# uclanlp/visualbert

Measured on NVIDIA H100. Metric: image-text pairs/sec fwd+bwd VisualBERT-base, higher is better.
Workload: dtype bf16

## Files before the change

visualbert_b200/csrc/vb_common.cuh:

```cuda
#pragma once

#include <cuda.h>
#include <cuda_bf16.h>
#include <cuda_runtime.h>
#include <stdint.h>
#include <stdio.h>

#include <atomic>

namespace vb {

typedef __nv_bfloat16 bf16;

extern std::atomic<long long> g_launches;
int num_sms();
constexpr int kMaxDevices = 64;
int current_device();
struct DetWs { void* ptr; long long bytes; };
DetWs det_ws();
int det_require(long long need, const char* what);
const unsigned long long* drop_offset();
template <typename K>
inline cudaError_t ensure_dyn_smem(K kern, int bytes, int (&cache)[kMaxDevices]) {
    const int d = current_device();
    if (cache[d] >= bytes) return cudaSuccess;
    cudaError_t e = cudaFuncSetAttribute(kern, cudaFuncAttributeMaxDynamicSharedMemorySize, bytes);
    if (e == cudaSuccess) cache[d] = bytes;
    return e;
}

enum { PROF_GEMM_FWD = 0, PROF_GEMM_DGRAD = 1, PROF_GEMM_WGRAD = 2, PROF_ATTN_FWD = 3, PROF_ATTN_DQ = 4, PROF_ATTN_DKV = 5,
       PROF_LN_FWD = 6, PROF_LN_BWD = 7, PROF_COLSUM = 8, PROF_EMBED = 9, PROF_OTHER = 10, PROF_NCAT = 11 };
#ifdef __CUDACC__
__device__ __forceinline__ void pdl_wait() { asm volatile("griddepcontrol.wait;" ::: "memory"); }
__device__ __forceinline__ void pdl_trigger() { asm volatile("griddepcontrol.launch_dependents;" ::: "memory"); }
template <typename... KArgs, typename... Args>
inline cudaError_t launch_pdl(void (*kernel)(KArgs...), dim3 grid, dim3 block, size_t smem, cudaStream_t st, Args&&... args) {
    cudaLaunchConfig_t cfg = {};
    cfg.gridDim = grid;
    cfg.blockDim = block;
    cfg.dynamicSmemBytes = smem;
    cfg.stream = st;
    cudaLaunchAttribute attr[1];
    attr[0].id = cudaLaunchAttributeProgrammaticStreamSerialization;
    attr[0].val.programmaticStreamSerializationAllowed = 1;
    cfg.attrs = attr;
    cfg.numAttrs = 1;
    return cudaLaunchKernelEx(&cfg, kernel, static_cast<KArgs>(args)...);
}
#endif

struct ProfScope {
    ProfScope(cudaStream_t st, int cat, double work, int launches);
    ~ProfScope();
    int slot;
    cudaStream_t st;
};

void set_error(const char* fmt, ...);
#define VB_CHECK_CUDA(expr)                                                                   \
    do {                                                                                      \
        cudaError_t _e = (expr);                                                              \
        if (_e != cudaSuccess) {                                                              \
            vb::set_error("%s:%d: %s -> %s", __FILE__, __LINE__, #expr, cudaGetErrorString(_e)); \
            return 1;                                                                         \
        }                                                                                     \
    } while (0)
#define VB_REQUIRE(cond, ...)                                                                 \
    do {                                                                                      \
        if (!(cond)) {                                                                        \
            vb::set_error(__VA_ARGS__);                                                       \
            return 2;                                                                         \
        }                                                                                     \
    } while (0)

#define VB_TRY_RC(expr)      \
    do {                     \
        int _rc = (expr);    \
        if (_rc) return _rc; \
    } while (0)

template <typename... T>
inline bool all_aligned16(const T*... p) {
    return ((reinterpret_cast<uintptr_t>(p) | ... | uintptr_t{0}) & 15) == 0;
}

__device__ __forceinline__ uint32_t smem_u32(const void* p) {
    return static_cast<uint32_t>(__cvta_generic_to_shared(p));
}

__device__ __forceinline__ float warp_sum(float v) {
#pragma unroll
    for (int o = 16; o > 0; o >>= 1) v += __shfl_xor_sync(0xffffffffu, v, o);
    return v;
}
__device__ __forceinline__ float warp_max(float v) {
#pragma unroll
    for (int o = 16; o > 0; o >>= 1) v = fmaxf(v, __shfl_xor_sync(0xffffffffu, v, o));
    return v;
}

__device__ __forceinline__ uint32_t pack_bf16x2(float lo, float hi) {
    __nv_bfloat162 h = __floats2bfloat162_rn(lo, hi);
    return *reinterpret_cast<uint32_t*>(&h);
}
__device__ __forceinline__ float2 unpack_bf16x2(uint32_t v) {
    __nv_bfloat162 h = *reinterpret_cast<__nv_bfloat162*>(&v);
    return __bfloat1622float2(h);
}

__device__ __forceinline__ float fast_ex2(float x) {
    float r;
    asm("ex2.approx.ftz.f32 %0, %1;" : "=f"(r) : "f"(x));
    return r;
}
__device__ __forceinline__ float fast_rcp(float x) {
    float r;
    asm("rcp.approx.ftz.f32 %0, %1;" : "=f"(r) : "f"(x));
    return r;
}

__device__ __forceinline__ float erfc_abs_sqrt2(float x, float& e) {
    const float ax = fabsf(x);
    e = fast_ex2(x * x * -0.72134752044448170f);
    const float t = fast_rcp(fmaf(0.23164189f, ax, 1.0f));
    float poly = fmaf(1.061405429f, t, -1.453152027f);
    poly = fmaf(poly, t, 1.421413741f);
    poly = fmaf(poly, t, -0.284496736f);
    poly = fmaf(poly, t, 0.254829592f);
    return poly * t * e;
}
__device__ __forceinline__ float gelu_fwd(float x) {
    float e;
    const float q = erfc_abs_sqrt2(x, e);
    const float hx = 0.5f * x, ha = fabsf(hx);
    return fmaf(-ha, q, hx + ha);
}
__device__ __forceinline__ void gelu_fwd_bwd(float x, float& g, float& gp) {
    float e;
    const float q = erfc_abs_sqrt2(x, e);
    const float cdf = 0.5f + copysignf(fmaf(-0.5f, q, 0.5f), x);
    g = x * cdf;
    gp = fmaf(x * e, 0.3989422804014327f, cdf);
}
__device__ __forceinline__ float gelu_bwd(float x) {
    float e;
    const float q = erfc_abs_sqrt2(x, e);
    const float cdf = 0.5f + copysignf(fmaf(-0.5f, q, 0.5f), x);
    return fmaf(x * e, 0.3989422804014327f, cdf);
}

__device__ __forceinline__ uint32_t mix32(uint32_t x) {
    x ^= x >> 16; x *= 0x7feb352du;
    x ^= x >> 15; x *= 0x846ca68bu;
    x ^= x >> 16;
    return x;
}
__device__ __forceinline__ uint32_t dropout_key(uint64_t seed, uint32_t stream) {
    return mix32(static_cast<uint32_t>(seed) ^ mix32(static_cast<uint32_t>(seed >> 32) + 0x9E3779B9u * (stream + 1u)));
}
struct DropQ { unsigned thr8; float scale; };
inline DropQ dropout_quantise(float p) {
    DropQ q;
    unsigned n = static_cast<unsigned>(p * 256.0f + 0.5f);
    if (n > 255u) n = 255u;
    q.thr8 = n;
    q.scale = p > 0.f ? 256.0f / (256.0f - static_cast<float>(n)) : 0.f;
    return q;
}
__device__ __forceinline__ uint32_t dropout_keep8_key(uint32_t key0, uint64_t elem8, uint32_t thr8) {
    const uint32_t key = key0 ^ (static_cast<uint32_t>(elem8 >> 31) * 0x27d4eb2fu);
    const uint32_t base = static_cast<uint32_t>(elem8) << 1;
    const uint32_t t4 = thr8 * 0x01010101u;
    const uint32_t m0 = __vcmpgeu4(mix32(base ^ key), t4) & 0x01010101u;
    const uint32_t m1 = __vcmpgeu4(mix32((base + 1u) ^ key), t4) & 0x01010101u;
    return ((m0 * 0x01020408u) >> 24) | (((m1 * 0x01020408u) >> 24) << 4);
}
__device__ __forceinline__ uint32_t dropout_keep8(uint64_t seed, uint32_t stream, uint64_t elem8, uint32_t thr8) {
    return dropout_keep8_key(dropout_key(seed, stream), elem8, thr8);
}

__device__ __forceinline__ void mbar_init(uint32_t bar, uint32_t count) {
    asm volatile("mbarrier.init.shared::cta.b64 [%0], %1;" ::"r"(bar), "r"(count) : "memory");
}
__device__ __forceinline__ void fence_barrier_init() {
    asm volatile("fence.mbarrier_init.release.cluster;" ::: "memory");
}
__device__ __forceinline__ void fence_proxy_async_smem() {
    asm volatile("fence.proxy.async.shared::cta;" ::: "memory");
}
__device__ __forceinline__ void mbar_arrive(uint32_t bar) {
    asm volatile("mbarrier.arrive.shared::cta.b64 _, [%0];" ::"r"(bar) : "memory");
}
__device__ __forceinline__ void mbar_arrive_expect_tx(uint32_t bar, uint32_t bytes) {
    asm volatile("mbarrier.arrive.expect_tx.shared::cta.b64 _, [%0], %1;" ::"r"(bar), "r"(bytes)
                 : "memory");
}
__device__ __forceinline__ bool mbar_try_wait(uint32_t bar, uint32_t parity) {
    uint32_t ok;
    asm volatile(
        "{\n"
        ".reg .pred p;\n"
        "mbarrier.try_wait.parity.shared::cta.b64 p, [%1], %2;\n"
        "selp.u32 %0, 1, 0, p;\n"
        "}\n"
        : "=r"(ok)
        : "r"(bar), "r"(parity)
        : "memory");
    return ok != 0;
}
__device__ __forceinline__ void mbar_wait(uint32_t bar, uint32_t parity) {
    if (mbar_try_wait(bar, parity)) return;
    const long long t0 = clock64();
    uint32_t spins = 0;
    while (!mbar_try_wait(bar, parity)) {
        if ((++spins & 0x3ffu) == 0 && clock64() - t0 > 4000000000ll) __trap();
    }
}

__device__ __forceinline__ void tma_prefetch_desc(const CUtensorMap* m) {
    asm volatile("prefetch.tensormap [%0];" ::"l"(reinterpret_cast<uint64_t>(m)) : "memory");
}
__device__ __forceinline__ void tma_load_2d(uint32_t smem_dst, const CUtensorMap* m, uint32_t bar,
                                            int c_inner, int c_outer) {
    asm volatile(
        "cp.async.bulk.tensor.2d.shared::cluster.global.mbarrier::complete_tx::bytes"
        " [%0], [%1, {%3, %4}], [%2];"
        ::"r"(smem_dst), "l"(reinterpret_cast<uint64_t>(m)), "r"(bar), "r"(c_inner), "r"(c_outer)
        : "memory");
}

__device__ __forceinline__ uint64_t wgmma_desc_sw128(uint32_t saddr, uint32_t lbo_bytes, uint32_t sbo_bytes) {
    return static_cast<uint64_t>((saddr & 0x3FFFFu) >> 4) | (static_cast<uint64_t>((lbo_bytes >> 4) & 0x3FFFu) << 16) |
           (static_cast<uint64_t>((sbo_bytes >> 4) & 0x3FFFu) << 32) | (1ull << 62);
}
__device__ __forceinline__ void wgmma_fence() { asm volatile("wgmma.fence.sync.aligned;" ::: "memory"); }
__device__ __forceinline__ void wgmma_commit() { asm volatile("wgmma.commit_group.sync.aligned;" ::: "memory"); }
template <int N>
__device__ __forceinline__ void wgmma_wait() { asm volatile("wgmma.wait_group.sync.aligned %0;" ::"n"(N) : "memory"); }
template <int TA, int TB>
__device__ __forceinline__ void wgmma_m64n128k16(float (&d)[64], uint64_t a_desc, uint64_t b_desc, uint32_t accumulate) {
    asm volatile(
        "{\n"
        ".reg .pred p;\n"
        "setp.ne.b32 p, %66, 0;\n"
        "wgmma.mma_async.sync.aligned.m64n128k16.f32.bf16.bf16 "
        "{%0, %1, %2, %3, %4, %5, %6, %7, %8, %9, %10, %11, %12, %13, %14, %15, %16, %17, %18, %19, %20, %21, %22, %23, %24, %25, %26, %27, %28, %29, %30, %31, %32, %33, %34, %35, %36, %37, %38, %39, %40, %41, %42, %43, %44, %45, %46, %47, %48, %49, %50, %51, %52, %53, %54, %55, %56, %57, %58, %59, %60, %61, %62, %63}, "
        "%64, %65, p, 1, 1, %67, %68;\n"
        "}\n"
        : "+f"(d[0]), "+f"(d[1]), "+f"(d[2]), "+f"(d[3]), "+f"(d[4]), "+f"(d[5]), "+f"(d[6]), "+f"(d[7]),
          "+f"(d[8]), "+f"(d[9]), "+f"(d[10]), "+f"(d[11]), "+f"(d[12]), "+f"(d[13]), "+f"(d[14]), "+f"(d[15]),
          "+f"(d[16]), "+f"(d[17]), "+f"(d[18]), "+f"(d[19]), "+f"(d[20]), "+f"(d[21]), "+f"(d[22]), "+f"(d[23]),
          "+f"(d[24]), "+f"(d[25]), "+f"(d[26]), "+f"(d[27]), "+f"(d[28]), "+f"(d[29]), "+f"(d[30]), "+f"(d[31]),
          "+f"(d[32]), "+f"(d[33]), "+f"(d[34]), "+f"(d[35]), "+f"(d[36]), "+f"(d[37]), "+f"(d[38]), "+f"(d[39]),
          "+f"(d[40]), "+f"(d[41]), "+f"(d[42]), "+f"(d[43]), "+f"(d[44]), "+f"(d[45]), "+f"(d[46]), "+f"(d[47]),
          "+f"(d[48]), "+f"(d[49]), "+f"(d[50]), "+f"(d[51]), "+f"(d[52]), "+f"(d[53]), "+f"(d[54]), "+f"(d[55]),
          "+f"(d[56]), "+f"(d[57]), "+f"(d[58]), "+f"(d[59]), "+f"(d[60]), "+f"(d[61]), "+f"(d[62]), "+f"(d[63])
        : "l"(a_desc), "l"(b_desc), "r"(accumulate), "n"(TA), "n"(TB));
}
template <int TA, int TB>
__device__ __forceinline__ void wgmma_m64n64k16_ss(float (&d)[32], uint64_t a_desc, uint64_t b_desc, uint32_t accumulate) {
    asm volatile(
        "{\n"
        ".reg .pred p;\n"
        "setp.ne.b32 p, %34, 0;\n"
        "wgmma.mma_async.sync.aligned.m64n64k16.f32.bf16.bf16 "
        "{%0, %1, %2, %3, %4, %5, %6, %7, %8, %9, %10, %11, %12, %13, %14, %15, %16, %17, %18, %19, %20, %21, %22, %23, %24, %25, %26, %27, %28, %29, %30, %31}, "
        "%32, %33, p, 1, 1, %35, %36;\n"
        "}\n"
        : "+f"(d[0]), "+f"(d[1]), "+f"(d[2]), "+f"(d[3]), "+f"(d[4]), "+f"(d[5]), "+f"(d[6]), "+f"(d[7]),
          "+f"(d[8]), "+f"(d[9]), "+f"(d[10]), "+f"(d[11]), "+f"(d[12]), "+f"(d[13]), "+f"(d[14]), "+f"(d[15]),
          "+f"(d[16]), "+f"(d[17]), "+f"(d[18]), "+f"(d[19]), "+f"(d[20]), "+f"(d[21]), "+f"(d[22]), "+f"(d[23]),
          "+f"(d[24]), "+f"(d[25]), "+f"(d[26]), "+f"(d[27]), "+f"(d[28]), "+f"(d[29]), "+f"(d[30]), "+f"(d[31])
        : "l"(a_desc), "l"(b_desc), "r"(accumulate), "n"(TA), "n"(TB));
}
template <int TB>
__device__ __forceinline__ void wgmma_m64n64k16_rs(float (&d)[32], const uint32_t (&a)[4], uint64_t b_desc, uint32_t accumulate) {
    asm volatile(
        "{\n"
        ".reg .pred p;\n"
        "setp.ne.b32 p, %37, 0;\n"
        "wgmma.mma_async.sync.aligned.m64n64k16.f32.bf16.bf16 "
        "{%0, %1, %2, %3, %4, %5, %6, %7, %8, %9, %10, %11, %12, %13, %14, %15, %16, %17, %18, %19, %20, %21, %22, %23, %24, %25, %26, %27, %28, %29, %30, %31}, "
        "{%32, %33, %34, %35}, %36, p, 1, 1, %38;\n"
        "}\n"
        : "+f"(d[0]), "+f"(d[1]), "+f"(d[2]), "+f"(d[3]), "+f"(d[4]), "+f"(d[5]), "+f"(d[6]), "+f"(d[7]),
          "+f"(d[8]), "+f"(d[9]), "+f"(d[10]), "+f"(d[11]), "+f"(d[12]), "+f"(d[13]), "+f"(d[14]), "+f"(d[15]),
          "+f"(d[16]), "+f"(d[17]), "+f"(d[18]), "+f"(d[19]), "+f"(d[20]), "+f"(d[21]), "+f"(d[22]), "+f"(d[23]),
          "+f"(d[24]), "+f"(d[25]), "+f"(d[26]), "+f"(d[27]), "+f"(d[28]), "+f"(d[29]), "+f"(d[30]), "+f"(d[31])
        : "r"(a[0]), "r"(a[1]), "r"(a[2]), "r"(a[3]), "l"(b_desc), "r"(accumulate), "n"(TB));
}
__device__ __forceinline__ bool elect_one() {
    uint32_t pred;
    asm volatile(
        "{\n"
        ".reg .pred P1;\n"
        "elect.sync _|P1, 0xffffffff;\n"
        "selp.u32 %0, 1, 0, P1;\n"
        "}\n"
        : "=r"(pred));
    return pred != 0;
}
template <int N>
__device__ __forceinline__ void reg_dec() { asm volatile("setmaxnreg.dec.sync.aligned.u32 %0;" ::"n"(N)); }
template <int N>
__device__ __forceinline__ void reg_inc() { asm volatile("setmaxnreg.inc.sync.aligned.u32 %0;" ::"n"(N)); }
__device__ __forceinline__ void named_bar_sync(int id, int nthreads) {
    asm volatile("bar.sync %0, %1;" ::"r"(id), "r"(nthreads) : "memory");
}

__device__ __forceinline__ uint4 ldg_v4(const void* p) {
    return __ldg(reinterpret_cast<const uint4*>(p));
}
__device__ __forceinline__ void stg_v4(void* p, uint4 v) { *reinterpret_cast<uint4*>(p) = v; }
__device__ __forceinline__ void ldg_v8(const void* p, uint32_t (&r)[8]) {
    const uint4 a = ldg_v4(p), b = ldg_v4(static_cast<const uint8_t*>(p) + 16);
    r[0] = a.x; r[1] = a.y; r[2] = a.z; r[3] = a.w; r[4] = b.x; r[5] = b.y; r[6] = b.z; r[7] = b.w;
}
__device__ __forceinline__ void stg_v8(void* p, const uint32_t (&r)[8]) {
    stg_v4(p, make_uint4(r[0], r[1], r[2], r[3]));
    stg_v4(static_cast<uint8_t*>(p) + 16, make_uint4(r[4], r[5], r[6], r[7]));
}
__device__ __forceinline__ void red_add_v4_f32(float* p, float a, float b, float c, float d) {
    asm volatile("red.global.add.v4.f32 [%0], {%1, %2, %3, %4};" ::"l"(p), "f"(a), "f"(b), "f"(c),
                 "f"(d)
                 : "memory");
}

}
```

visualbert_b200/csrc/vb_gemm.cu:

```cuda
#include <stdarg.h>
#include <stdio.h>
#include <stdlib.h>
#include <string.h>

#include <atomic>
#include <mutex>
#include <vector>

#include "../../include/vbert_b200.h"
#include "vb_common.cuh"

namespace vb {

static thread_local char g_err[1024] = "";
std::atomic<long long> g_launches{0};

void set_error(const char* fmt, ...) {
    va_list ap;
    va_start(ap, fmt);
    vsnprintf(g_err, sizeof(g_err), fmt, ap);
    va_end(ap);
}
const char* get_error() { return g_err; }

static thread_local void* g_det_ptr = nullptr;
static thread_local long long g_det_bytes = 0;
DetWs det_ws() { return DetWs{g_det_ptr, g_det_bytes}; }
int det_require(long long need, const char* what) {
    VB_REQUIRE(g_det_ptr == nullptr || need <= g_det_bytes,
               "%s: deterministic mode needs %lld bytes of workspace, %lld are set (vb_deterministic_workspace_bytes)", what, need,
               g_det_bytes);
    return 0;
}
static thread_local const unsigned long long* g_drop_offset = nullptr;
const unsigned long long* drop_offset() { return g_drop_offset; }

struct ProfRec { cudaEvent_t e0, e1; int cat; double work; int launches; };
static bool g_prof_on = false;
static std::vector<ProfRec> g_prof;
static std::vector<ProfRec> g_prof_pool;
static std::mutex g_prof_mu;

ProfScope::ProfScope(cudaStream_t s, int cat, double work, int launches) : slot(-1), st(s) {
    g_launches.fetch_add(launches);
    if (!g_prof_on) return;
    cudaStreamCaptureStatus cs = cudaStreamCaptureStatusNone;
    if (cudaStreamIsCapturing(s, &cs) != cudaSuccess || cs != cudaStreamCaptureStatusNone) return;
    std::lock_guard<std::mutex> lk(g_prof_mu);
    ProfRec r;
    if (!g_prof_pool.empty()) { r = g_prof_pool.back(); g_prof_pool.pop_back(); }
    else { cudaEventCreate(&r.e0); cudaEventCreate(&r.e1); }
    r.cat = cat; r.work = work; r.launches = launches;
    cudaEventRecord(r.e0, st);
    g_prof.push_back(r);
    slot = static_cast<int>(g_prof.size()) - 1;
}
ProfScope::~ProfScope() {
    if (slot < 0) return;
    std::lock_guard<std::mutex> lk(g_prof_mu);
    cudaEventRecord(g_prof[slot].e1, st);
}

constexpr int BLOCK_M = 128;
constexpr int BLOCK_K = 64;
constexpr int WGMMA_K = 16;
constexpr int kStages = 4;
constexpr int kEpiWarps = 8;
constexpr int kThreads = 128 + kEpiWarps * 32;
constexpr int kAtomBytes = 64 * BLOCK_K * 2;

template <int BLOCK_N>
struct Cfg {
    static constexpr int A_BYTES = BLOCK_M * BLOCK_K * 2;
    static constexpr int B_BYTES = BLOCK_N * BLOCK_K * 2;
    static constexpr int STAGE_BYTES = A_BYTES + B_BYTES;
    static constexpr int ACC_LD = BLOCK_N + 4;
    static constexpr int RING_BYTES = kStages * STAGE_BYTES > BLOCK_M * ACC_LD * 4 ? kStages * STAGE_BYTES : BLOCK_M * ACC_LD * 4;
    static constexpr int BAR_OFF = RING_BYTES;
    static constexpr int NUM_BARS = 2 * kStages;
    static constexpr int BIAS_OFF = BAR_OFF + NUM_BARS * 8;
    static constexpr int SMEM_BYTES = BIAS_OFF + BLOCK_N * 4 + 1024;
    static_assert(SMEM_BYTES <= 227 * 1024, "shared memory per block");
};

struct GemmParams {
    int M, N, K;
    int splits;
    void* D; long long ldd;
    const float* bias;
    const bf16* addend; long long ld_add;
    int epilogue;
    const bf16* aux_in;
    bf16* aux_out; long long ld_aux;
    float drop_scale;
    unsigned drop_thresh16;
    unsigned long long drop_seed;
    unsigned drop_stream;
    int m_fast;
    union {
        float* delta_out;
        const unsigned long long* drop_offset;
    };
    int delta_seq;
};
bool gemm_gp_tiled_ok(int M, int N);
bool gemm_delta_ok(int M, int N);

struct TileCoord {
    int m_blk, n_blk, kb_begin, kb_end;
};
__device__ __forceinline__ TileCoord decode_tile(int t, int n_blocks, int splits, int k_blocks, int m_blocks, bool m_fast) {
    TileCoord c;
    const int tiles = m_blocks * n_blocks;
    const int split = t / tiles;
    const int mn = t - split * tiles;
    if (m_fast) {
        c.m_blk = mn % m_blocks;
        c.n_blk = mn / m_blocks;
    } else {
        c.n_blk = mn % n_blocks;
        c.m_blk = mn / n_blocks;
    }
    c.kb_begin = static_cast<int>(static_cast<long long>(split) * k_blocks / splits);
    c.kb_end = static_cast<int>(static_cast<long long>(split + 1) * k_blocks / splits);
    return c;
}

__device__ __forceinline__ void load16_bf16(const bf16* p, float (&f)[16]) {
    uint32_t r[8];
    ldg_v8(p, r);
#pragma unroll
    for (int i = 0; i < 8; ++i) {
        const float2 t = unpack_bf16x2(r[i]);
        f[2 * i] = t.x;
        f[2 * i + 1] = t.y;
    }
}
__device__ __forceinline__ void store16_bf16(bf16* p, const float (&f)[16]) {
    uint32_t r[8];
#pragma unroll
    for (int i = 0; i < 8; ++i) r[i] = pack_bf16x2(f[2 * i], f[2 * i + 1]);
    stg_v8(p, r);
}

enum { EPI_GENERIC = 0, EPI_BIAS = 1, EPI_RESID = 2, EPI_DROP_RESID = 3, EPI_GELU_FWD = 4, EPI_DGELU_BWD = 5, EPI_GELU_FWD_T = 6,
       EPI_DGELU_BWD_T = 7, EPI_DELTA = 8, EPI_GELU_ONLY = 9, EPI_SLAB = 10, EPI_GENERIC_OFF = 11 };
__host__ __device__ constexpr bool epi_is_generic(int e) { return e == EPI_GENERIC || e == EPI_GENERIC_OFF; }
__host__ __device__ constexpr bool epi_is_gelu(int e) { return e == EPI_GELU_FWD || e == EPI_GELU_FWD_T; }
__host__ __device__ constexpr bool epi_is_dgelu(int e) { return e == EPI_DGELU_BWD || e == EPI_DGELU_BWD_T; }

template <bool OUT_F32, int EPI = EPI_GENERIC, bool TO_REGS = false>
__device__ __forceinline__ void epilogue16(const GemmParams& p, int row, int col, const float* sbias, const uint32_t (&ex)[8],
                                           float (&x)[16], uint32_t* o0 = nullptr, uint32_t* o1 = nullptr) {
    if (sbias != nullptr) {
#pragma unroll
        for (int i = 0; i < 4; ++i) {
            const float4 b = *reinterpret_cast<const float4*>(sbias + 4 * i);
            x[4 * i] += b.x; x[4 * i + 1] += b.y; x[4 * i + 2] += b.z; x[4 * i + 3] += b.w;
        }
    }
    if constexpr (OUT_F32) {
        float* d = reinterpret_cast<float*>(p.D) + static_cast<long long>(row) * p.ldd + col;
#pragma unroll
        for (int i = 0; i < 4; ++i) red_add_v4_f32(d + 4 * i, x[4 * i], x[4 * i + 1], x[4 * i + 2], x[4 * i + 3]);
    } else {
        constexpr bool kGeneric = epi_is_generic(EPI);
        if (EPI == EPI_DROP_RESID || (kGeneric && p.drop_scale != 0.0f)) {
            const unsigned long long e8 =
                (static_cast<unsigned long long>(row) * static_cast<unsigned>(p.N) + col) >> 3;
#pragma unroll
            for (int h = 0; h < 2; ++h) {
                const uint32_t keep = dropout_keep8(EPI == EPI_GENERIC_OFF ? p.drop_seed + *p.drop_offset : p.drop_seed, p.drop_stream, e8 + h,
                                                    p.drop_thresh16);
#pragma unroll
                for (int i = 0; i < 8; ++i) x[8 * h + i] = ((keep >> i) & 1u) ? x[8 * h + i] * p.drop_scale : 0.0f;
            }
        }
        if (EPI == EPI_RESID || EPI == EPI_DROP_RESID || (kGeneric && p.addend != nullptr)) {
#pragma unroll
            for (int i = 0; i < 8; ++i) {
                const float2 t = unpack_bf16x2(ex[i]);
                x[2 * i] += t.x;
                x[2 * i + 1] += t.y;
            }
        }
        bf16* d = reinterpret_cast<bf16*>(p.D) + static_cast<long long>(row) * p.ldd + col;
        if (EPI == EPI_GELU_ONLY) {
#pragma unroll
            for (int i = 0; i < 16; ++i) {
                float gp;
                gelu_fwd_bwd(x[i], x[i], gp);
            }
        } else if (epi_is_gelu(EPI) || (kGeneric && p.epilogue == VB_EPI_GELU)) {
            float gp[16];
#pragma unroll
            for (int i = 0; i < 16; ++i) gelu_fwd_bwd(x[i], x[i], gp[i]);
            if constexpr (TO_REGS) {
#pragma unroll
                for (int i = 0; i < 8; ++i) { o0[i] = pack_bf16x2(gp[2 * i], gp[2 * i + 1]); o1[i] = pack_bf16x2(x[2 * i], x[2 * i + 1]); }
                return;
            }
            store16_bf16(d, gp);
            d = p.aux_out + static_cast<long long>(row) * p.ld_aux + col;
        } else if (epi_is_dgelu(EPI) || (kGeneric && p.epilogue == VB_EPI_DGELU)) {
#pragma unroll
            for (int i = 0; i < 8; ++i) {
                const float2 t = unpack_bf16x2(ex[i]);
                x[2 * i] *= t.x;
                x[2 * i + 1] *= t.y;
            }
        }
        if constexpr (TO_REGS) {
#pragma unroll
            for (int i = 0; i < 8; ++i) o0[i] = pack_bf16x2(x[2 * i], x[2 * i + 1]);
            return;
        }
        store16_bf16(d, x);
    }
}

template <bool A_MN, bool B_MN, int BLOCK_N, bool OUT_F32, int EPI = EPI_GENERIC>
__global__ void __launch_bounds__(kThreads, 1)
gemm_wgmma_kernel(const __grid_constant__ CUtensorMap tmA, const __grid_constant__ CUtensorMap tmB, const GemmParams p) {
    using C = Cfg<BLOCK_N>;
    static_assert(BLOCK_N % 128 == 0, "64 x 128 wgmma pieces");
    static_assert(!(EPI == EPI_GELU_FWD_T || EPI == EPI_DGELU_BWD_T) || BLOCK_N == 256, "tile-native gelu' is defined on 256-wide tiles");
    extern __shared__ uint8_t smem_raw[];
    const uint32_t raw = smem_u32(smem_raw);
    const uint32_t base = (raw + 1023u) & ~1023u;
    uint8_t* smem = smem_raw + (base - raw);

    const int warp = threadIdx.x >> 5;
    const int lane = threadIdx.x & 31;

    auto a_tile = [&](int s) { return base + s * C::STAGE_BYTES; };
    auto b_tile = [&](int s) { return base + s * C::STAGE_BYTES + C::A_BYTES; };
    auto full_bar = [&](int s) { return base + C::BAR_OFF + 8 * s; };
    auto empty_bar = [&](int s) { return base + C::BAR_OFF + 8 * (kStages + s); };

    if (threadIdx.x == 0) {
        tma_prefetch_desc(&tmA);
        tma_prefetch_desc(&tmB);
        for (int s = 0; s < kStages; ++s) {
            mbar_init(full_bar(s), 1);
            mbar_init(empty_bar(s), 2);
        }
        fence_barrier_init();
    }
    __syncthreads();
    pdl_trigger();
    pdl_wait();

    const int m_blocks = (p.M + BLOCK_M - 1) / BLOCK_M;
    const int n_blocks = (p.N + BLOCK_N - 1) / BLOCK_N;
    const int k_blocks = (p.K + BLOCK_K - 1) / BLOCK_K;
    const TileCoord tc = decode_tile(blockIdx.x, n_blocks, p.splits, k_blocks, m_blocks, p.m_fast != 0);

    if (warp < 4) {
        reg_dec<40>();
        if (warp == 0) {
            int stage = 0;
            uint32_t phase = 0;
            for (int kb = tc.kb_begin; kb < tc.kb_end; ++kb) {
                mbar_wait(empty_bar(stage), phase ^ 1u);
                if (elect_one()) {
                    mbar_arrive_expect_tx(full_bar(stage), C::STAGE_BYTES);
                    if constexpr (!A_MN) {
                        tma_load_2d(a_tile(stage), &tmA, full_bar(stage), kb * BLOCK_K, tc.m_blk * BLOCK_M);
                    } else {
#pragma unroll
                        for (int i = 0; i < BLOCK_M / 64; ++i)
                            tma_load_2d(a_tile(stage) + i * kAtomBytes, &tmA, full_bar(stage), tc.m_blk * BLOCK_M + i * 64, kb * BLOCK_K);
                    }
                    if constexpr (!B_MN) {
                        tma_load_2d(b_tile(stage), &tmB, full_bar(stage), kb * BLOCK_K, tc.n_blk * BLOCK_N);
                    } else {
#pragma unroll
                        for (int i = 0; i < BLOCK_N / 64; ++i)
                            tma_load_2d(b_tile(stage) + i * kAtomBytes, &tmB, full_bar(stage), tc.n_blk * BLOCK_N + i * 64, kb * BLOCK_K);
                    }
                }
                __syncwarp();
                if (++stage == kStages) { stage = 0; phase ^= 1u; }
            }
        }
        return;
    }
    reg_inc<232>();

    const int wg = (warp >> 2) - 1;
    const int et = threadIdx.x - 128;
    float* sbias = reinterpret_cast<float*>(smem + C::BIAS_OFF);
    const bool has_bias = p.bias != nullptr;
    if (has_bias) {
        const bool mine = tc.kb_begin == 0;
        for (int i = et; i < BLOCK_N; i += kEpiWarps * 32) {
            const int col = tc.n_blk * BLOCK_N + i;
            sbias[i] = (mine && col < p.N) ? __ldg(p.bias + col) : 0.f;
        }
    }
    constexpr int NH = BLOCK_N / 128;
    constexpr uint32_t a_kstep = A_MN ? WGMMA_K * 128 : WGMMA_K * 2;
    constexpr uint32_t b_kstep = B_MN ? WGMMA_K * 128 : WGMMA_K * 2;
    float acc[NH][64];
    {
        int stage = 0, prev = 0;
        uint32_t phase = 0;
        for (int kb = tc.kb_begin; kb < tc.kb_end; ++kb) {
            mbar_wait(full_bar(stage), phase);
            const uint32_t a0 = a_tile(stage) + wg * 8192, b0 = b_tile(stage);
            wgmma_fence();
#pragma unroll
            for (int k = 0; k < BLOCK_K / WGMMA_K; ++k) {
                const uint64_t ad = wgmma_desc_sw128(a0 + k * a_kstep, kAtomBytes, 1024);
#pragma unroll
                for (int h = 0; h < NH; ++h)
                    wgmma_m64n128k16<A_MN ? 1 : 0, B_MN ? 1 : 0>(acc[h], ad, wgmma_desc_sw128(b0 + h * 16384 + k * b_kstep, kAtomBytes, 1024),
                                                                 (kb > tc.kb_begin || k > 0) ? 1u : 0u);
            }
            wgmma_commit();
            wgmma_wait<1>();
            if (kb > tc.kb_begin && (threadIdx.x & 127) == 0) mbar_arrive(empty_bar(prev));
            prev = stage;
            if (++stage == kStages) { stage = 0; phase ^= 1u; }
        }
        wgmma_wait<0>();
    }

    const int ew = warp - 4;
    const int q = ew & 3, half = ew >> 2;
    const int col0 = tc.n_blk * BLOCK_N + half * (BLOCK_N / 2);
    constexpr int NCH = BLOCK_N / 2 / 16;
    constexpr int RPI = 32 / NCH;
    constexpr bool kRowPerLane = EPI == EPI_DELTA;
    auto wrow_of = [&](int j) { return kRowPerLane ? lane : RPI * j + lane % RPI; };
    auto chunk_of = [&](int j) { return kRowPerLane ? j : lane / RPI; };
    const long long gp_warp_off =
        ((((static_cast<long long>(tc.m_blk >> 1) * n_blocks + tc.n_blk) * 2 + (tc.m_blk & 1)) * kEpiWarps + ew) * NCH) * 512;
    auto gp_off = [&](int j) { return gp_warp_off + chunk_of(j) * 512 + wrow_of(j) * 16; };
    constexpr bool kEx = !OUT_F32 && EPI != EPI_BIAS && !epi_is_gelu(EPI) && EPI != EPI_GELU_ONLY;
    uint32_t ex[kEx ? NCH : 1][8];
    if constexpr (kEx) {
        constexpr bool kWantAdd = EPI == EPI_RESID || EPI == EPI_DROP_RESID || EPI == EPI_DELTA;
        const int row0 = tc.m_blk * BLOCK_M + q * 32 + wrow_of(0), c0 = col0 + chunk_of(0) * 16;
        const bf16* exb = nullptr;
        long long ex_step = 0;
        if (kWantAdd || (epi_is_generic(EPI) && p.addend != nullptr)) {
            exb = p.addend + static_cast<long long>(row0) * p.ld_add + c0;
            ex_step = kRowPerLane ? 16 : RPI * p.ld_add;
        } else if (EPI == EPI_DGELU_BWD || (epi_is_generic(EPI) && p.epilogue == VB_EPI_DGELU)) {
            exb = p.aux_in + static_cast<long long>(row0) * p.ld_aux + c0;
            ex_step = kRowPerLane ? 16 : RPI * p.ld_aux;
        } else if (EPI == EPI_DGELU_BWD_T) {
            exb = p.aux_in + gp_off(0);
            ex_step = kRowPerLane ? 512 : RPI * 16;
        }
#pragma unroll
        for (int j = 0; j < NCH; ++j)
            if (exb != nullptr && tc.m_blk * BLOCK_M + q * 32 + wrow_of(j) < p.M && col0 + chunk_of(j) * 16 < p.N) ldg_v8(exb + j * ex_step, ex[j]);
    }

    named_bar_sync(1, kEpiWarps * 32);
    float* sacc = reinterpret_cast<float*>(smem);
    {
        const int r0 = wg * 64 + ((warp & 3) << 4) + (lane >> 2);
#pragma unroll
        for (int h = 0; h < NH; ++h)
#pragma unroll
            for (int j = 0; j < 16; ++j)
#pragma unroll
                for (int i = 0; i < 2; ++i)
                    *reinterpret_cast<float2*>(sacc + (r0 + 8 * i) * C::ACC_LD + h * 128 + j * 8 + 2 * (lane & 3)) =
                        make_float2(acc[h][4 * j + 2 * i], acc[h][4 * j + 2 * i + 1]);
    }
    named_bar_sync(1, kEpiWarps * 32);

    [[maybe_unused]] float hsum = 0.f;
#pragma unroll
    for (int k = 0; k < NCH; ++k) {
        const int lrow = q * 32 + wrow_of(k), cc = half * (BLOCK_N / 2) + chunk_of(k) * 16;
        const int row = tc.m_blk * BLOCK_M + lrow;
        const int col = tc.n_blk * BLOCK_N + cc;
        if (row < p.M && col < p.N) {
            float x[16];
#pragma unroll
            for (int i = 0; i < 4; ++i) {
                const float4 v = *reinterpret_cast<const float4*>(sacc + lrow * C::ACC_LD + cc + 4 * i);
                x[4 * i] = v.x; x[4 * i + 1] = v.y; x[4 * i + 2] = v.z; x[4 * i + 3] = v.w;
            }
            const float* sb = has_bias ? sbias + cc : nullptr;
            const uint32_t (&e)[8] = ex[kEx ? k : 0];
            if constexpr (EPI == EPI_GELU_FWD_T) {
                uint32_t o0[8], o1[8];
                epilogue16<OUT_F32, EPI, true>(p, row, col, sb, e, x, o0, o1);
                stg_v8(reinterpret_cast<bf16*>(p.D) + gp_off(k), o0);
                stg_v8(p.aux_out + static_cast<long long>(row) * p.ld_aux + col, o1);
            } else if constexpr (EPI == EPI_SLAB) {
                float* d = reinterpret_cast<float*>(p.D) + (static_cast<long long>(blockIdx.x / (m_blocks * n_blocks)) * p.M + row) * p.ldd + col;
#pragma unroll
                for (int i = 0; i < 4; ++i) *reinterpret_cast<float4*>(d + 4 * i) = make_float4(x[4 * i], x[4 * i + 1], x[4 * i + 2], x[4 * i + 3]);
            } else if constexpr (EPI == EPI_DELTA) {
                uint32_t o0[8];
                epilogue16<OUT_F32, EPI, true>(p, row, col, sb, e, x, o0);
                stg_v8(reinterpret_cast<bf16*>(p.D) + static_cast<long long>(row) * p.ldd + col, o0);
#pragma unroll
                for (int i = 0; i < 8; ++i) {
                    const float2 a = unpack_bf16x2(o0[i]), b = unpack_bf16x2(e[i]);
                    hsum = fmaf(a.x, b.x, fmaf(a.y, b.y, hsum));
                }
            } else {
                epilogue16<OUT_F32, EPI>(p, row, col, sb, e, x);
            }
        }
        if constexpr (EPI == EPI_DELTA) {
            if ((k & 3) == 3) {
                const int c4 = col - 48;
                if (row < p.M && c4 < p.N) {
                    const int bi = row / p.delta_seq, si = row - bi * p.delta_seq;
                    p.delta_out[(static_cast<long long>(bi) * (p.N >> 6) + (c4 >> 6)) * p.delta_seq + si] = hsum;
                }
                hsum = 0.f;
            }
        }
    }
}

typedef CUresult (*EncodeTiledFn)(CUtensorMap*, CUtensorMapDataType, cuuint32_t, void*, const cuuint64_t*,
                                  const cuuint64_t*, const cuuint32_t*, const cuuint32_t*,
                                  CUtensorMapInterleave, CUtensorMapSwizzle, CUtensorMapL2promotion,
                                  CUtensorMapFloatOOBfill);

static EncodeTiledFn get_encode_fn() {
    static EncodeTiledFn fn = nullptr;
    static bool tried = false;
    if (!tried) {
        tried = true;
        void* sym = nullptr;
        cudaDriverEntryPointQueryResult qres;
        if (cudaGetDriverEntryPoint("cuTensorMapEncodeTiled", &sym, cudaEnableDefault, &qres) == cudaSuccess &&
            qres == cudaDriverEntryPointSuccess)
            fn = reinterpret_cast<EncodeTiledFn>(sym);
    }
    return fn;
}

struct TmapKey {
    const void* ptr; uint64_t d0, d1, d2, s0, s1; uint32_t b0, b1, b2, rank; int dev;
    bool operator==(const TmapKey& o) const {
        return ptr == o.ptr && d0 == o.d0 && d1 == o.d1 && d2 == o.d2 && s0 == o.s0 && s1 == o.s1 && b0 == o.b0 && b1 == o.b1 && b2 == o.b2 &&
               rank == o.rank && dev == o.dev;
    }
};
struct TmapSlot { TmapKey key; CUtensorMap map; bool used; };
constexpr int kTmapSlots = 4096;
static thread_local std::vector<TmapSlot>* g_tmap_cache = nullptr;

static int encode_tmap_cached(CUtensorMap* m, const void* ptr, uint32_t rank, const cuuint64_t* dims, const cuuint64_t* strides,
                              const cuuint32_t* box) {
    TmapKey k;
    memset(&k, 0, sizeof(k));
    k.ptr = ptr; k.rank = rank; k.dev = current_device();
    k.d0 = dims[0]; k.d1 = dims[1]; k.d2 = rank > 2 ? dims[2] : 1;
    k.s0 = strides[0]; k.s1 = rank > 2 ? strides[1] : 0;
    k.b0 = box[0]; k.b1 = box[1]; k.b2 = rank > 2 ? box[2] : 1;
    uint64_t h = reinterpret_cast<uintptr_t>(ptr) * 0x9E3779B97F4A7C15ull;
    h ^= (k.d0 * 31 + k.d1) * 0xBF58476D1CE4E5B9ull + k.d2 * 1315423911ull + k.s0 * 2654435761ull + k.s1 * 40503ull;
    h ^= (static_cast<uint64_t>(k.b1) << 20) ^ (static_cast<uint64_t>(k.b0) << 8) ^ k.b2 ^ (static_cast<uint64_t>(k.dev) << 40);
    h ^= h >> 29;
    if (g_tmap_cache == nullptr) { g_tmap_cache = new std::vector<TmapSlot>(kTmapSlots); for (auto& sl : *g_tmap_cache) sl.used = false; }
    TmapSlot& sl = (*g_tmap_cache)[h & (kTmapSlots - 1)];
    if (sl.used && sl.key == k) { *m = sl.map; return 0; }
    EncodeTiledFn fn = get_encode_fn();
    VB_REQUIRE(fn != nullptr, "cuTensorMapEncodeTiled unavailable (driver too old / no GPU?)");
    cuuint32_t estr[3] = {1, 1, 1};
    CUresult r = fn(m, CU_TENSOR_MAP_DATA_TYPE_BFLOAT16, rank, const_cast<void*>(ptr), dims, strides, box, estr,
                    CU_TENSOR_MAP_INTERLEAVE_NONE, CU_TENSOR_MAP_SWIZZLE_128B, CU_TENSOR_MAP_L2_PROMOTION_L2_256B,
                    CU_TENSOR_MAP_FLOAT_OOB_FILL_NONE);
    VB_REQUIRE(r == CUDA_SUCCESS, "cuTensorMapEncodeTiled (rank %u) failed with CUresult %d", rank, static_cast<int>(r));
    sl.key = k; sl.map = *m; sl.used = true;
    return 0;
}

int make_tmap_bf16(CUtensorMap* m, const void* ptr, uint64_t inner, uint64_t outer, uint64_t ld_elems,
                   uint32_t box_outer) {
    VB_REQUIRE((reinterpret_cast<uintptr_t>(ptr) & 15) == 0, "TMA operand not 16-byte aligned");
    VB_REQUIRE((ld_elems * 2) % 16 == 0, "TMA operand row stride must be a multiple of 8 elements");
    cuuint64_t dims[2] = {inner, outer};
    cuuint64_t strides[1] = {ld_elems * 2};
    cuuint32_t box[2] = {64, box_outer};
    return encode_tmap_cached(m, ptr, 2, dims, strides, box);
}

int current_device() {
    int dev = 0;
    cudaGetDevice(&dev);
    return (dev < 0 || dev >= kMaxDevices) ? 0 : dev;
}

int num_sms() {
    static int n[kMaxDevices] = {0};
    const int dev = current_device();
    if (n[dev] == 0) {
        int v = 0;
        cudaDeviceGetAttribute(&v, cudaDevAttrMultiProcessorCount, dev);
        n[dev] = v > 0 ? v : 132;
    }
    return n[dev];
}

template <bool A_MN, bool B_MN, int BLOCK_N, bool OUT_F32, int EPI = EPI_GENERIC>
static int launch(const CUtensorMap& ta, const CUtensorMap& tb, const GemmParams& p, cudaStream_t st) {
    using C = Cfg<BLOCK_N>;
    auto kern = gemm_wgmma_kernel<A_MN, B_MN, BLOCK_N, OUT_F32, EPI>;
    static int configured[kMaxDevices] = {0};
    VB_CHECK_CUDA(ensure_dyn_smem(kern, C::SMEM_BYTES, configured));
    const long long tiles = static_cast<long long>((p.M + BLOCK_M - 1) / BLOCK_M) * ((p.N + BLOCK_N - 1) / BLOCK_N) * p.splits;
    VB_REQUIRE(tiles < (1LL << 31), "vb_gemm: too many tiles");
    {
        ProfScope ps(st, OUT_F32 ? PROF_GEMM_WGRAD : (B_MN ? PROF_GEMM_DGRAD : PROF_GEMM_FWD), 2.0 * p.M * p.N * p.K, 1);
        VB_CHECK_CUDA(launch_pdl(kern, dim3(static_cast<unsigned>(tiles)), dim3(kThreads), C::SMEM_BYTES, st, ta, tb, p));
    }
    VB_CHECK_CUDA(cudaGetLastError());
    return 0;
}

int wgrad_splits(long long tiles, int k_blocks) {
    constexpr int kCtaCost = 4;
    const long long sms = num_sms();
    int best = 1;
    long long best_cost = -1;
    for (int s = 1; s <= k_blocks && s <= 32; ++s) {
        const long long cost = (tiles * s + sms - 1) / sms * ((k_blocks + s - 1) / s + kCtaCost);
        if (best_cost < 0 || cost < best_cost) { best = s; best_cost = cost; }
    }
    return best;
}

__global__ void __launch_bounds__(256)
splitk_reduce_kernel(const float* __restrict__ slab, int splits, int M, int N, const float* __restrict__ bias, float* __restrict__ D,
                     long long ldd) {
    const long long n4 = static_cast<long long>(M) * N / 4, plane = static_cast<long long>(M) * N;
    for (long long i = static_cast<long long>(blockIdx.x) * blockDim.x + threadIdx.x; i < n4; i += static_cast<long long>(gridDim.x) * blockDim.x) {
        const long long e = 4 * i;
        const int row = static_cast<int>(e / N), col = static_cast<int>(e - static_cast<long long>(row) * N);
        float4 a = *reinterpret_cast<const float4*>(slab + e);
        if (bias != nullptr) { a.x += bias[col]; a.y += bias[col + 1]; a.z += bias[col + 2]; a.w += bias[col + 3]; }
        for (int s = 1; s < splits; ++s) {
            const float4 b = *reinterpret_cast<const float4*>(slab + s * plane + e);
            a.x += b.x; a.y += b.y; a.z += b.z; a.w += b.w;
        }
        float4* d = reinterpret_cast<float4*>(D + static_cast<long long>(row) * ldd + col);
        float4 o = *d;
        o.x += a.x; o.y += a.y; o.z += a.z; o.w += a.w;
        *d = o;
    }
}

static bool use_bn256(int N) { return N >= 256 && ((N + 255) / 256 * 256 - N) * 8 <= N; }
long long gemm_tiles(int M, int N) {
    const bool bn256 = use_bn256(N);
    return static_cast<long long>((M + BLOCK_M - 1) / BLOCK_M) * ((N + (bn256 ? 255 : 127)) / (bn256 ? 256 : 128));
}
int gemm_k_blocks(int K) { return (K + BLOCK_K - 1) / BLOCK_K; }

bool gemm_delta_ok(int M, int N) {
    const int n_pad256 = (N + 255) / 256 * 256;
    return M >= 256 && N >= 256 && N % 64 == 0 && (n_pad256 - N) * 8 <= N;
}
bool gemm_gp_tiled_ok(int M, int N) {
    return M >= 256 && M % 256 == 0 && N % 256 == 0;
}

int gemm(const vb_gemm_args& a, cudaStream_t st) {
    VB_REQUIRE(a.M > 0 && a.N > 0 && a.K > 0, "vb_gemm: empty problem M=%d N=%d K=%d", a.M, a.N, a.K);
    VB_REQUIRE(a.N % 16 == 0, "vb_gemm: N=%d must be a multiple of 16", a.N);
    VB_REQUIRE(a.A && a.B && a.D, "vb_gemm: null operand");
    VB_REQUIRE(a.ldd % 16 == 0 && (reinterpret_cast<uintptr_t>(a.D) & 31) == 0, "vb_gemm: D must be 32-byte aligned with ldd a multiple of 16");
    VB_REQUIRE(!a.addend || (a.ld_add % 16 == 0 && (reinterpret_cast<uintptr_t>(a.addend) & 31) == 0), "vb_gemm: addend must be 32-byte aligned with ld a multiple of 16");
    VB_REQUIRE((!a.aux_in && !a.aux_out) || a.ld_aux % 16 == 0, "vb_gemm: ld_aux must be a multiple of 16");
    VB_REQUIRE((reinterpret_cast<uintptr_t>(a.aux_in) & 31) == 0 && (reinterpret_cast<uintptr_t>(a.aux_out) & 31) == 0,
               "vb_gemm: aux_in / aux_out must be 32-byte aligned");
    VB_REQUIRE(a.epilogue == VB_EPI_NONE || a.epilogue == VB_EPI_GELU || a.epilogue == VB_EPI_DGELU || a.epilogue == VB_EPI_GELU_FWD,
               "vb_gemm: unknown epilogue %d", a.epilogue);
    VB_REQUIRE(a.epilogue != VB_EPI_GELU || a.aux_out, "vb_gemm: GELU epilogue needs aux_out");
    VB_REQUIRE(a.epilogue != VB_EPI_DGELU || a.aux_in, "vb_gemm: DGELU epilogue needs aux_in");
    VB_REQUIRE(a.epilogue == VB_EPI_NONE || (!a.addend && a.dropout_p == 0.0f),
               "vb_gemm: the GELU / DGELU / GELU_FWD epilogues take no dropout and no addend");
    VB_REQUIRE(a.epilogue != VB_EPI_GELU_FWD || (!a.a_mn_major && !a.b_mn_major && !a.d_fp32 && !a.aux_in && !a.aux_out),
               "vb_gemm: the GELU_FWD epilogue needs K-major A and B and a bf16 D, and takes no aux_in / aux_out");
    VB_REQUIRE(!a.d_fp32 || (a.epilogue == VB_EPI_NONE && !a.addend && a.dropout_p == 0.0f),
               "vb_gemm: fp32-accumulate output supports bias only");
    VB_REQUIRE(a.dropout_p >= 0.0f && a.dropout_p < 1.0f, "vb_gemm: dropout_p out of range");
    VB_REQUIRE(!a.delta_out || (gemm_delta_ok(a.M, a.N) && a.delta_ctx && a.delta_seq > 0 && a.M % a.delta_seq == 0 && !a.d_fp32 &&
                                !a.a_mn_major && a.b_mn_major && !a.bias && !a.addend && a.dropout_p == 0.0f && a.epilogue == VB_EPI_NONE &&
                                (reinterpret_cast<uintptr_t>(a.delta_ctx) & 31) == 0),
               "vb_gemm: delta_out needs a plain bf16 input-gradient GEMM (b_mn_major, no bias / addend / dropout) and vb_gemm_delta_ok(M, N)");
    VB_REQUIRE(!a.gp_tiled || (gemm_gp_tiled_ok(a.M, a.N) && !a.d_fp32 && !a.a_mn_major && (a.epilogue == VB_EPI_GELU || a.epilogue == VB_EPI_DGELU)),
               "vb_gemm: gp_tiled needs a GELU / DGELU epilogue and vb_gemm_gp_tiled_ok(M, N)");
    VB_REQUIRE(!a.gp_tiled || a.epilogue != VB_EPI_DGELU || a.b_mn_major,
               "vb_gemm: gp_tiled with the DGELU epilogue needs an MN-major B (the input-gradient GEMM)");
    VB_REQUIRE(!a.gp_tiled || a.epilogue != VB_EPI_GELU || !a.b_mn_major, "vb_gemm: gp_tiled with the GELU epilogue needs a K-major B");

    GemmParams p;
    memset(&p, 0, sizeof(p));
    p.M = a.M; p.N = a.N; p.K = a.K;
    p.D = a.D; p.ldd = a.ldd;
    p.bias = a.bias;
    p.addend = static_cast<const bf16*>(a.addend); p.ld_add = a.ld_add;
    p.epilogue = a.epilogue;
    p.aux_in = static_cast<const bf16*>(a.aux_in);
    p.aux_out = static_cast<bf16*>(a.aux_out);
    p.ld_aux = a.ld_aux;
    if (a.delta_out) {
        p.addend = static_cast<const bf16*>(a.delta_ctx); p.ld_add = a.N;
        p.delta_out = a.delta_out; p.delta_seq = a.delta_seq;
    }
    p.m_fast = (a.M + BLOCK_M - 1) / BLOCK_M < (a.N + 255) / 256 ? 1 : 0;
    const unsigned long long* const off = a.dropout_p > 0.0f ? drop_offset() : nullptr;
    if (a.dropout_p > 0.0f) {
        const DropQ q = dropout_quantise(a.dropout_p);
        p.drop_scale = q.scale;
        p.drop_thresh16 = q.thr8;
        p.drop_seed = a.dropout_seed;
        p.drop_stream = a.dropout_stream;
        if (off != nullptr) p.drop_offset = off;
    }

    const bool bn256 = use_bn256(a.N);
    VB_REQUIRE(!a.delta_out || bn256, "vb_gemm: delta_out needs 256-wide tiles");
    p.splits = a.d_fp32 ? wgrad_splits(gemm_tiles(a.M, a.N), gemm_k_blocks(a.K)) : 1;
    const DetWs det = det_ws();
    if (a.d_fp32 && p.splits > 1 && det.ptr != nullptr) {
        const long long plane = static_cast<long long>(a.M) * a.N * 4;
        if (!(a.a_mn_major && a.b_mn_major)) p.splits = 1;
        while (p.splits > 1 && p.splits * plane > det.bytes) --p.splits;
    }
    const bool slab = a.d_fp32 && p.splits > 1 && det.ptr != nullptr;

    CUtensorMap ta, tb;
    int rc;
    if (!a.a_mn_major) rc = make_tmap_bf16(&ta, a.A, a.K, a.M, a.lda, BLOCK_M);
    else               rc = make_tmap_bf16(&ta, a.A, a.M, a.K, a.lda, BLOCK_K);
    if (rc) return rc;
    if (!a.b_mn_major) rc = make_tmap_bf16(&tb, a.B, a.K, a.N, a.ldb, bn256 ? 256 : 128);
    else               rc = make_tmap_bf16(&tb, a.B, a.N, a.K, a.ldb, BLOCK_K);
    if (rc) return rc;

    if (slab) {
        GemmParams q = p;
        q.D = det.ptr; q.ldd = a.N; q.bias = nullptr;
        const int rc2 = bn256 ? launch<true, true, 256, true, EPI_SLAB>(ta, tb, q, st) : launch<true, true, 128, true, EPI_SLAB>(ta, tb, q, st);
        if (rc2) return rc2;
        const long long n4 = static_cast<long long>(a.M) * a.N / 4;
        long long blocks = (n4 + 255) / 256;
        if (blocks > num_sms() * 8) blocks = num_sms() * 8;
        {
            ProfScope ps(st, PROF_GEMM_WGRAD, 0.0, 1);
            splitk_reduce_kernel<<<static_cast<int>(blocks), 256, 0, st>>>(static_cast<const float*>(det.ptr), p.splits, a.M, a.N, a.bias,
                                                                           static_cast<float*>(a.D), a.ldd);
        }
        VB_CHECK_CUDA(cudaGetLastError());
        return 0;
    }
    if (off != nullptr) {
#define VB_DISPATCH_OFF(AM, BM) \
    (bn256 ? launch<AM, BM, 256, false, EPI_GENERIC_OFF>(ta, tb, p, st) : launch<AM, BM, 128, false, EPI_GENERIC_OFF>(ta, tb, p, st))
        if (!a.a_mn_major && !a.b_mn_major) return VB_DISPATCH_OFF(false, false);
        if (!a.a_mn_major && a.b_mn_major) return VB_DISPATCH_OFF(false, true);
        if (a.a_mn_major && a.b_mn_major) return VB_DISPATCH_OFF(true, true);
        return VB_DISPATCH_OFF(true, false);
#undef VB_DISPATCH_OFF
    }
    if (a.epilogue == VB_EPI_GELU_FWD)
        return bn256 ? launch<false, false, 256, false, EPI_GELU_ONLY>(ta, tb, p, st) : launch<false, false, 128, false, EPI_GELU_ONLY>(ta, tb, p, st);
    if (bn256 && !a.d_fp32) {
        const bool drop = a.dropout_p > 0.0f, add = a.addend != nullptr;
        int epi = EPI_GENERIC;
        if (a.epilogue == VB_EPI_GELU) epi = a.gp_tiled ? EPI_GELU_FWD_T : EPI_GELU_FWD;
        else if (a.epilogue == VB_EPI_DGELU) epi = a.gp_tiled ? EPI_DGELU_BWD_T : EPI_DGELU_BWD;
        else epi = add ? (drop ? EPI_DROP_RESID : EPI_RESID) : (drop ? EPI_GENERIC : EPI_BIAS);
        if (a.delta_out) epi = EPI_DELTA;
        if (!a.a_mn_major && !a.b_mn_major) {
            switch (epi) {
                case EPI_BIAS: return launch<false, false, 256, false, EPI_BIAS>(ta, tb, p, st);
                case EPI_RESID: return launch<false, false, 256, false, EPI_RESID>(ta, tb, p, st);
                case EPI_DROP_RESID: return launch<false, false, 256, false, EPI_DROP_RESID>(ta, tb, p, st);
                case EPI_GELU_FWD: return launch<false, false, 256, false, EPI_GELU_FWD>(ta, tb, p, st);
                case EPI_GELU_FWD_T: return launch<false, false, 256, false, EPI_GELU_FWD_T>(ta, tb, p, st);
                default: return launch<false, false, 256, false>(ta, tb, p, st);
            }
        }
        if (!a.a_mn_major && a.b_mn_major) {
            switch (epi) {
                case EPI_BIAS: return launch<false, true, 256, false, EPI_BIAS>(ta, tb, p, st);
                case EPI_RESID: return launch<false, true, 256, false, EPI_RESID>(ta, tb, p, st);
                case EPI_DGELU_BWD: return launch<false, true, 256, false, EPI_DGELU_BWD>(ta, tb, p, st);
                case EPI_DELTA: return launch<false, true, 256, false, EPI_DELTA>(ta, tb, p, st);
                case EPI_DGELU_BWD_T: return launch<false, true, 256, false, EPI_DGELU_BWD_T>(ta, tb, p, st);
                default: return launch<false, true, 256, false>(ta, tb, p, st);
            }
        }
    }

#define VB_DISPATCH(AM, BM, F32)                                         \
    (bn256 ? launch<AM, BM, 256, F32>(ta, tb, p, st) : launch<AM, BM, 128, F32>(ta, tb, p, st))
    if (!a.d_fp32) {
        if (!a.a_mn_major && !a.b_mn_major) return VB_DISPATCH(false, false, false);
        if (!a.a_mn_major && a.b_mn_major) return VB_DISPATCH(false, true, false);
        if (a.a_mn_major && a.b_mn_major) return VB_DISPATCH(true, true, false);
        return VB_DISPATCH(true, false, false);
    } else {
        if (!a.a_mn_major && !a.b_mn_major) return VB_DISPATCH(false, false, true);
        if (!a.a_mn_major && a.b_mn_major) return VB_DISPATCH(false, true, true);
        if (a.a_mn_major && a.b_mn_major) return VB_DISPATCH(true, true, true);
        return VB_DISPATCH(true, false, true);
    }
#undef VB_DISPATCH
}

}

extern "C" {
int vb_abi_version(void) { return VB_ABI_VERSION; }
const char* vb_last_error(void) { return vb::get_error(); }
int64_t vb_launch_count(void) { return vb::g_launches.load(); }
void vb_profile_enable(int on) {
    std::lock_guard<std::mutex> lk(vb::g_prof_mu);
    vb::g_prof_on = on != 0;
}
int vb_profile_read(double* ms, double* work, int64_t* launches) {
    if (cudaDeviceSynchronize() != cudaSuccess) { vb::set_error("vb_profile_read: device sync failed"); return 1; }
    std::lock_guard<std::mutex> lk(vb::g_prof_mu);
    for (int c = 0; c < vb::PROF_NCAT; ++c) { ms[c] = 0; work[c] = 0; launches[c] = 0; }
    for (auto& r : vb::g_prof) {
        float t = 0.f;
        cudaEventElapsedTime(&t, r.e0, r.e1);
        ms[r.cat] += t; work[r.cat] += r.work; launches[r.cat] += r.launches;
        vb::g_prof_pool.push_back(r);
    }
    vb::g_prof.clear();
    return 0;
}
int vb_set_deterministic(void* workspace, int64_t bytes) {
    if (workspace != nullptr && (bytes <= 0 || (reinterpret_cast<uintptr_t>(workspace) & 255) != 0)) {
        vb::set_error("vb_set_deterministic: the workspace must be 256-byte aligned and bytes > 0 (got %p, %lld)", workspace,
                      static_cast<long long>(bytes));
        return 2;
    }
    vb::g_det_ptr = workspace;
    vb::g_det_bytes = workspace != nullptr ? bytes : 0;
    return 0;
}
int vb_set_dropout_offset(const uint64_t* offset) {
    if ((reinterpret_cast<uintptr_t>(offset) & 7) != 0) {
        vb::set_error("vb_set_dropout_offset: the offset must be 8-byte aligned (got %p)", static_cast<const void*>(offset));
        return 2;
    }
    vb::g_drop_offset = reinterpret_cast<const unsigned long long*>(offset);
    return 0;
}
int vb_gemm_delta_ok(int32_t M, int32_t N) { return vb::gemm_delta_ok(M, N) ? 1 : 0; }
int vb_gemm_gp_tiled_ok(int32_t M, int32_t N) { return vb::gemm_gp_tiled_ok(M, N) ? 1 : 0; }
int vb_gemm(const vb_gemm_args* args, void* stream) {
    if (!args) { vb::set_error("vb_gemm: null args"); return 2; }
    return vb::gemm(*args, static_cast<cudaStream_t>(stream));
}
}
```

Measured before the change: 4315.

## Route GEMM epilogue through shared memory with TMA loads/stores and n256 wgmma

```diff
diff --git a/visualbert_b200/csrc/vb_common.cuh b/visualbert_b200/csrc/vb_common.cuh
--- a/visualbert_b200/csrc/vb_common.cuh
+++ b/visualbert_b200/csrc/vb_common.cuh
@@ -230,6 +230,35 @@
         : "memory");
 }
 
+__device__ __forceinline__ void tma_store_2d(const CUtensorMap* m, uint32_t smem_src, int c_inner, int c_outer) {
+    asm volatile("cp.async.bulk.tensor.2d.global.shared::cta.bulk_group [%0, {%2, %3}], [%1];"
+                 ::"l"(reinterpret_cast<uint64_t>(m)), "r"(smem_src), "r"(c_inner), "r"(c_outer)
+                 : "memory");
+}
+__device__ __forceinline__ void bulk_load(uint32_t smem_dst, const void* src, uint32_t bytes, uint32_t bar) {
+    asm volatile("cp.async.bulk.shared::cluster.global.mbarrier::complete_tx::bytes [%0], [%1], %2, [%3];"
+                 ::"r"(smem_dst), "l"(reinterpret_cast<uint64_t>(src)), "r"(bytes), "r"(bar)
+                 : "memory");
+}
+__device__ __forceinline__ void bulk_store(void* dst, uint32_t smem_src, uint32_t bytes) {
+    asm volatile("cp.async.bulk.global.shared::cta.bulk_group [%0], [%1], %2;"
+                 ::"l"(reinterpret_cast<uint64_t>(dst)), "r"(smem_src), "r"(bytes)
+                 : "memory");
+}
+__device__ __forceinline__ void bulk_commit() { asm volatile("cp.async.bulk.commit_group;" ::: "memory"); }
+__device__ __forceinline__ void bulk_wait_read0() { asm volatile("cp.async.bulk.wait_group.read 0;" ::: "memory"); }
+
+__device__ __forceinline__ void ldmatrix_x4(uint32_t addr, uint32_t (&r)[4]) {
+    asm volatile("ldmatrix.sync.aligned.m8n8.x4.shared.b16 {%0, %1, %2, %3}, [%4];"
+                 : "=r"(r[0]), "=r"(r[1]), "=r"(r[2]), "=r"(r[3])
+                 : "r"(addr)
+                 : "memory");
+}
+__device__ __forceinline__ void stmatrix_x4(uint32_t addr, const uint32_t (&r)[4]) {
+    asm volatile("stmatrix.sync.aligned.m8n8.x4.shared.b16 [%0], {%1, %2, %3, %4};" ::"r"(addr), "r"(r[0]), "r"(r[1]), "r"(r[2]), "r"(r[3])
+                 : "memory");
+}
+
 __device__ __forceinline__ uint64_t wgmma_desc_sw128(uint32_t saddr, uint32_t lbo_bytes, uint32_t sbo_bytes) {
     return static_cast<uint64_t>((saddr & 0x3FFFFu) >> 4) | (static_cast<uint64_t>((lbo_bytes >> 4) & 0x3FFFu) << 16) |
            (static_cast<uint64_t>((sbo_bytes >> 4) & 0x3FFFu) << 32) | (1ull << 62);
@@ -259,6 +288,34 @@
         : "l"(a_desc), "l"(b_desc), "r"(accumulate), "n"(TA), "n"(TB));
 }
 template <int TA, int TB>
+__device__ __forceinline__ void wgmma_m64n256k16(float (&d)[128], uint64_t a_desc, uint64_t b_desc, uint32_t accumulate) {
+    asm volatile(
+        "{\n"
+        ".reg .pred p;\n"
+        "setp.ne.b32 p, %130, 0;\n"
+        "wgmma.mma_async.sync.aligned.m64n256k16.f32.bf16.bf16 "
+        "{%0, %1, %2, %3, %4, %5, %6, %7, %8, %9, %10, %11, %12, %13, %14, %15, %16, %17, %18, %19, %20, %21, %22, %23, %24, %25, %26, %27, %28, %29, %30, %31, %32, %33, %34, %35, %36, %37, %38, %39, %40, %41, %42, %43, %44, %45, %46, %47, %48, %49, %50, %51, %52, %53, %54, %55, %56, %57, %58, %59, %60, %61, %62, %63, %64, %65, %66, %67, %68, %69, %70, %71, %72, %73, %74, %75, %76, %77, %78, %79, %80, %81, %82, %83, %84, %85, %86, %87, %88, %89, %90, %91, %92, %93, %94, %95, %96, %97, %98, %99, %100, %101, %102, %103, %104, %105, %106, %107, %108, %109, %110, %111, %112, %113, %114, %115, %116, %117, %118, %119, %120, %121, %122, %123, %124, %125, %126, %127}, "
+        "%128, %129, p, 1, 1, %131, %132;\n"
+        "}\n"
+        : "+f"(d[0]), "+f"(d[1]), "+f"(d[2]), "+f"(d[3]), "+f"(d[4]), "+f"(d[5]), "+f"(d[6]), "+f"(d[7]),
+          "+f"(d[8]), "+f"(d[9]), "+f"(d[10]), "+f"(d[11]), "+f"(d[12]), "+f"(d[13]), "+f"(d[14]), "+f"(d[15]),
+          "+f"(d[16]), "+f"(d[17]), "+f"(d[18]), "+f"(d[19]), "+f"(d[20]), "+f"(d[21]), "+f"(d[22]), "+f"(d[23]),
+          "+f"(d[24]), "+f"(d[25]), "+f"(d[26]), "+f"(d[27]), "+f"(d[28]), "+f"(d[29]), "+f"(d[30]), "+f"(d[31]),
+          "+f"(d[32]), "+f"(d[33]), "+f"(d[34]), "+f"(d[35]), "+f"(d[36]), "+f"(d[37]), "+f"(d[38]), "+f"(d[39]),
+          "+f"(d[40]), "+f"(d[41]), "+f"(d[42]), "+f"(d[43]), "+f"(d[44]), "+f"(d[45]), "+f"(d[46]), "+f"(d[47]),
+          "+f"(d[48]), "+f"(d[49]), "+f"(d[50]), "+f"(d[51]), "+f"(d[52]), "+f"(d[53]), "+f"(d[54]), "+f"(d[55]),
+          "+f"(d[56]), "+f"(d[57]), "+f"(d[58]), "+f"(d[59]), "+f"(d[60]), "+f"(d[61]), "+f"(d[62]), "+f"(d[63]),
+          "+f"(d[64]), "+f"(d[65]), "+f"(d[66]), "+f"(d[67]), "+f"(d[68]), "+f"(d[69]), "+f"(d[70]), "+f"(d[71]),
+          "+f"(d[72]), "+f"(d[73]), "+f"(d[74]), "+f"(d[75]), "+f"(d[76]), "+f"(d[77]), "+f"(d[78]), "+f"(d[79]),
+          "+f"(d[80]), "+f"(d[81]), "+f"(d[82]), "+f"(d[83]), "+f"(d[84]), "+f"(d[85]), "+f"(d[86]), "+f"(d[87]),
+          "+f"(d[88]), "+f"(d[89]), "+f"(d[90]), "+f"(d[91]), "+f"(d[92]), "+f"(d[93]), "+f"(d[94]), "+f"(d[95]),
+          "+f"(d[96]), "+f"(d[97]), "+f"(d[98]), "+f"(d[99]), "+f"(d[100]), "+f"(d[101]), "+f"(d[102]), "+f"(d[103]),
+          "+f"(d[104]), "+f"(d[105]), "+f"(d[106]), "+f"(d[107]), "+f"(d[108]), "+f"(d[109]), "+f"(d[110]), "+f"(d[111]),
+          "+f"(d[112]), "+f"(d[113]), "+f"(d[114]), "+f"(d[115]), "+f"(d[116]), "+f"(d[117]), "+f"(d[118]), "+f"(d[119]),
+          "+f"(d[120]), "+f"(d[121]), "+f"(d[122]), "+f"(d[123]), "+f"(d[124]), "+f"(d[125]), "+f"(d[126]), "+f"(d[127])
+        : "l"(a_desc), "l"(b_desc), "r"(accumulate), "n"(TA), "n"(TB));
+}
+template <int TA, int TB>
 __device__ __forceinline__ void wgmma_m64n64k16_ss(float (&d)[32], uint64_t a_desc, uint64_t b_desc, uint32_t accumulate) {
     asm volatile(
         "{\n"
diff --git a/visualbert_b200/csrc/vb_gemm.cu b/visualbert_b200/csrc/vb_gemm.cu
--- a/visualbert_b200/csrc/vb_gemm.cu
+++ b/visualbert_b200/csrc/vb_gemm.cu
@@ -76,9 +76,14 @@
     static constexpr int STAGE_BYTES = A_BYTES + B_BYTES;
     static constexpr int ACC_LD = BLOCK_N + 4;
     static constexpr int RING_BYTES = kStages * STAGE_BYTES > BLOCK_M * ACC_LD * 4 ? kStages * STAGE_BYTES : BLOCK_M * ACC_LD * 4;
+    static constexpr int PIECE = 16384;
+    static constexpr int PIECES_PER_SLOT = STAGE_BYTES / PIECE;
+    static constexpr int OPND = BLOCK_N / 64;
+    static constexpr int OPND_SLOTS = (OPND + PIECES_PER_SLOT - 1) / PIECES_PER_SLOT;
+    static_assert(STAGE_BYTES % PIECE == 0 && 3 * OPND <= kStages * PIECES_PER_SLOT, "operand + two output tiles fit the ring");
     static constexpr int BAR_OFF = RING_BYTES;
-    static constexpr int NUM_BARS = 2 * kStages;
-    static constexpr int BIAS_OFF = BAR_OFF + NUM_BARS * 8;
+    static constexpr int NUM_BARS = 2 * kStages + 1;
+    static constexpr int BIAS_OFF = (BAR_OFF + NUM_BARS * 8 + 15) / 16 * 16;
     static constexpr int SMEM_BYTES = BIAS_OFF + BLOCK_N * 4 + 1024;
     static_assert(SMEM_BYTES <= 227 * 1024, "shared memory per block");
 };
@@ -126,105 +131,37 @@
     return c;
 }
 
-__device__ __forceinline__ void load16_bf16(const bf16* p, float (&f)[16]) {
-    uint32_t r[8];
-    ldg_v8(p, r);
-#pragma unroll
-    for (int i = 0; i < 8; ++i) {
-        const float2 t = unpack_bf16x2(r[i]);
-        f[2 * i] = t.x;
-        f[2 * i + 1] = t.y;
-    }
-}
-__device__ __forceinline__ void store16_bf16(bf16* p, const float (&f)[16]) {
-    uint32_t r[8];
-#pragma unroll
-    for (int i = 0; i < 8; ++i) r[i] = pack_bf16x2(f[2 * i], f[2 * i + 1]);
-    stg_v8(p, r);
-}
-
 enum { EPI_GENERIC = 0, EPI_BIAS = 1, EPI_RESID = 2, EPI_DROP_RESID = 3, EPI_GELU_FWD = 4, EPI_DGELU_BWD = 5, EPI_GELU_FWD_T = 6,
        EPI_DGELU_BWD_T = 7, EPI_DELTA = 8, EPI_GELU_ONLY = 9, EPI_SLAB = 10, EPI_GENERIC_OFF = 11 };
 __host__ __device__ constexpr bool epi_is_generic(int e) { return e == EPI_GENERIC || e == EPI_GENERIC_OFF; }
 __host__ __device__ constexpr bool epi_is_gelu(int e) { return e == EPI_GELU_FWD || e == EPI_GELU_FWD_T; }
 __host__ __device__ constexpr bool epi_is_dgelu(int e) { return e == EPI_DGELU_BWD || e == EPI_DGELU_BWD_T; }
-
-template <bool OUT_F32, int EPI = EPI_GENERIC, bool TO_REGS = false>
-__device__ __forceinline__ void epilogue16(const GemmParams& p, int row, int col, const float* sbias, const uint32_t (&ex)[8],
-                                           float (&x)[16], uint32_t* o0 = nullptr, uint32_t* o1 = nullptr) {
-    if (sbias != nullptr) {
-#pragma unroll
-        for (int i = 0; i < 4; ++i) {
-            const float4 b = *reinterpret_cast<const float4*>(sbias + 4 * i);
-            x[4 * i] += b.x; x[4 * i + 1] += b.y; x[4 * i + 2] += b.z; x[4 * i + 3] += b.w;
-        }
-    }
-    if constexpr (OUT_F32) {
-        float* d = reinterpret_cast<float*>(p.D) + static_cast<long long>(row) * p.ldd + col;
-#pragma unroll
-        for (int i = 0; i < 4; ++i) red_add_v4_f32(d + 4 * i, x[4 * i], x[4 * i + 1], x[4 * i + 2], x[4 * i + 3]);
-    } else {
-        constexpr bool kGeneric = epi_is_generic(EPI);
-        if (EPI == EPI_DROP_RESID || (kGeneric && p.drop_scale != 0.0f)) {
-            const unsigned long long e8 =
-                (static_cast<unsigned long long>(row) * static_cast<unsigned>(p.N) + col) >> 3;
-#pragma unroll
-            for (int h = 0; h < 2; ++h) {
-                const uint32_t keep = dropout_keep8(EPI == EPI_GENERIC_OFF ? p.drop_seed + *p.drop_offset : p.drop_seed, p.drop_stream, e8 + h,
-                                                    p.drop_thresh16);
-#pragma unroll
-                for (int i = 0; i < 8; ++i) x[8 * h + i] = ((keep >> i) & 1u) ? x[8 * h + i] * p.drop_scale : 0.0f;
-            }
-        }
-        if (EPI == EPI_RESID || EPI == EPI_DROP_RESID || (kGeneric && p.addend != nullptr)) {
-#pragma unroll
-            for (int i = 0; i < 8; ++i) {
-                const float2 t = unpack_bf16x2(ex[i]);
-                x[2 * i] += t.x;
-                x[2 * i + 1] += t.y;
-            }
-        }
-        bf16* d = reinterpret_cast<bf16*>(p.D) + static_cast<long long>(row) * p.ldd + col;
-        if (EPI == EPI_GELU_ONLY) {
-#pragma unroll
-            for (int i = 0; i < 16; ++i) {
-                float gp;
-                gelu_fwd_bwd(x[i], x[i], gp);
-            }
-        } else if (epi_is_gelu(EPI) || (kGeneric && p.epilogue == VB_EPI_GELU)) {
-            float gp[16];
-#pragma unroll
-            for (int i = 0; i < 16; ++i) gelu_fwd_bwd(x[i], x[i], gp[i]);
-            if constexpr (TO_REGS) {
-#pragma unroll
-                for (int i = 0; i < 8; ++i) { o0[i] = pack_bf16x2(gp[2 * i], gp[2 * i + 1]); o1[i] = pack_bf16x2(x[2 * i], x[2 * i + 1]); }
-                return;
-            }
-            store16_bf16(d, gp);
-            d = p.aux_out + static_cast<long long>(row) * p.ld_aux + col;
-        } else if (epi_is_dgelu(EPI) || (kGeneric && p.epilogue == VB_EPI_DGELU)) {
-#pragma unroll
-            for (int i = 0; i < 8; ++i) {
-                const float2 t = unpack_bf16x2(ex[i]);
-                x[2 * i] *= t.x;
-                x[2 * i + 1] *= t.y;
-            }
-        }
-        if constexpr (TO_REGS) {
-#pragma unroll
-            for (int i = 0; i < 8; ++i) o0[i] = pack_bf16x2(x[2 * i], x[2 * i + 1]);
-            return;
-        }
-        store16_bf16(d, x);
-    }
+__host__ __device__ constexpr bool epi_may_read(int e) {
+    return e == EPI_RESID || e == EPI_DROP_RESID || epi_is_dgelu(e) || e == EPI_DELTA || epi_is_generic(e);
+}
+__device__ __forceinline__ bool epi_reads(int e, const GemmParams& p) {
+    return e == EPI_RESID || e == EPI_DROP_RESID || epi_is_dgelu(e) || e == EPI_DELTA ||
+           (epi_is_generic(e) && (p.addend != nullptr || p.epilogue == VB_EPI_DGELU));
+}
+
+template <int BLOCK_N, int TA, int TB>
+__device__ __forceinline__ void wgmma_tile(float (&acc)[BLOCK_N / 2], uint64_t ad, uint64_t bd, uint32_t accumulate) {
+    if constexpr (BLOCK_N == 256) wgmma_m64n256k16<TA, TB>(acc, ad, bd, accumulate);
+    else wgmma_m64n128k16<TA, TB>(acc, ad, bd, accumulate);
+}
+
+__device__ __forceinline__ uint32_t tn_byte(int row, int col) {
+    return ((((col >> 7) * 4 + (row >> 5)) * 8 + ((col & 127) >> 4)) * 512 + (row & 31) * 16 + (col & 15)) * 2;
 }
 
 template <bool A_MN, bool B_MN, int BLOCK_N, bool OUT_F32, int EPI = EPI_GENERIC>
 __global__ void __launch_bounds__(kThreads, 1)
-gemm_wgmma_kernel(const __grid_constant__ CUtensorMap tmA, const __grid_constant__ CUtensorMap tmB, const GemmParams p) {
+gemm_wgmma_kernel(const __grid_constant__ CUtensorMap tmA, const __grid_constant__ CUtensorMap tmB, const GemmParams p,
+                  const __grid_constant__ CUtensorMap tmD, const __grid_constant__ CUtensorMap tmX, const __grid_constant__ CUtensorMap tmE) {
     using C = Cfg<BLOCK_N>;
-    static_assert(BLOCK_N % 128 == 0, "64 x 128 wgmma pieces");
+    static_assert(BLOCK_N == 128 || BLOCK_N == 256, "64 x 128 / 64 x 256 wgmma tiles");
     static_assert(!(EPI == EPI_GELU_FWD_T || EPI == EPI_DGELU_BWD_T) || BLOCK_N == 256, "tile-native gelu' is defined on 256-wide tiles");
+    static_assert(!(EPI == EPI_DELTA) || BLOCK_N == 256, "EPI_DELTA: four whole heads per tile");
     extern __shared__ uint8_t smem_raw[];
     const uint32_t raw = smem_u32(smem_raw);
     const uint32_t base = (raw + 1023u) & ~1023u;
@@ -237,6 +174,7 @@
     auto b_tile = [&](int s) { return base + s * C::STAGE_BYTES + C::A_BYTES; };
     auto full_bar = [&](int s) { return base + C::BAR_OFF + 8 * s; };
     auto empty_bar = [&](int s) { return base + C::BAR_OFF + 8 * (kStages + s); };
+    const uint32_t opnd_bar = base + C::BAR_OFF + 8 * (2 * kStages);
 
     if (threadIdx.x == 0) {
         tma_prefetch_desc(&tmA);
@@ -245,6 +183,7 @@
             mbar_init(full_bar(s), 1);
             mbar_init(empty_bar(s), 2);
         }
+        mbar_init(opnd_bar, 1);
         fence_barrier_init();
     }
     __syncthreads();
@@ -255,6 +194,11 @@
     const int n_blocks = (p.N + BLOCK_N - 1) / BLOCK_N;
     const int k_blocks = (p.K + BLOCK_K - 1) / BLOCK_K;
     const TileCoord tc = decode_tile(blockIdx.x, n_blocks, p.splits, k_blocks, m_blocks, p.m_fast != 0);
+    const int n_kb = tc.kb_end - tc.kb_begin;
+    auto piece_addr = [&](int k) {
+        return base + ((n_kb + k / C::PIECES_PER_SLOT) % kStages) * C::STAGE_BYTES + (k % C::PIECES_PER_SLOT) * C::PIECE;
+    };
+    const long long tn_tile = ((static_cast<long long>(tc.m_blk >> 1) * n_blocks + tc.n_blk) * 2 + (tc.m_blk & 1)) * (BLOCK_M * BLOCK_N);
 
     if (warp < 4) {
         reg_dec<40>();
@@ -283,6 +227,28 @@
                 __syncwarp();
                 if (++stage == kStages) { stage = 0; phase ^= 1u; }
             }
+            if constexpr (!OUT_F32 && epi_may_read(EPI)) {
+                if (epi_reads(EPI, p)) {
+                    for (int t = 0; t < C::OPND_SLOTS; ++t) {
+                        mbar_wait(empty_bar(stage), phase ^ 1u);
+                        if (++stage == kStages) { stage = 0; phase ^= 1u; }
+                    }
+                    if (elect_one()) {
+                        mbar_arrive_expect_tx(opnd_bar, C::OPND * C::PIECE);
+                        if (EPI == EPI_DGELU_BWD_T) {
+                            const uint8_t* src = reinterpret_cast<const uint8_t*>(p.aux_in) + tn_tile * 2;
+#pragma unroll
+                            for (int k = 0; k < C::OPND; ++k) bulk_load(piece_addr(k), src + k * C::PIECE, C::PIECE, opnd_bar);
+                        } else {
+                            tma_prefetch_desc(&tmE);
+#pragma unroll
+                            for (int k = 0; k < C::OPND; ++k)
+                                tma_load_2d(piece_addr(k), &tmE, opnd_bar, tc.n_blk * BLOCK_N + 64 * k, tc.m_blk * BLOCK_M);
+                        }
+                    }
+                    __syncwarp();
+                }
+            }
         }
         return;
     }
@@ -299,10 +265,9 @@
             sbias[i] = (mine && col < p.N) ? __ldg(p.bias + col) : 0.f;
         }
     }
-    constexpr int NH = BLOCK_N / 128;
     constexpr uint32_t a_kstep = A_MN ? WGMMA_K * 128 : WGMMA_K * 2;
     constexpr uint32_t b_kstep = B_MN ? WGMMA_K * 128 : WGMMA_K * 2;
-    float acc[NH][64];
+    float acc[BLOCK_N / 2];
     {
         int stage = 0, prev = 0;
         uint32_t phase = 0;
@@ -311,13 +276,10 @@
             const uint32_t a0 = a_tile(stage) + wg * 8192, b0 = b_tile(stage);
             wgmma_fence();
 #pragma unroll
-            for (int k = 0; k < BLOCK_K / WGMMA_K; ++k) {
-                const uint64_t ad = wgmma_desc_sw128(a0 + k * a_kstep, kAtomBytes, 1024);
-#pragma unroll
-                for (int h = 0; h < NH; ++h)
-                    wgmma_m64n128k16<A_MN ? 1 : 0, B_MN ? 1 : 0>(acc[h], ad, wgmma_desc_sw128(b0 + h * 16384 + k * b_kstep, kAtomBytes, 1024),
-                                                                 (kb > tc.kb_begin || k > 0) ? 1u : 0u);
-            }
+            for (int k = 0; k < BLOCK_K / WGMMA_K; ++k)
+                wgmma_tile<BLOCK_N, A_MN ? 1 : 0, B_MN ? 1 : 0>(acc, wgmma_desc_sw128(a0 + k * a_kstep, kAtomBytes, 1024),
+                                                              wgmma_desc_sw128(b0 + k * b_kstep, kAtomBytes, 1024),
+                                                              (kb > tc.kb_begin || k > 0) ? 1u : 0u);
             wgmma_commit();
             wgmma_wait<1>();
             if (kb > tc.kb_begin && (threadIdx.x & 127) == 0) mbar_arrive(empty_bar(prev));
@@ -326,102 +288,209 @@
         }
         wgmma_wait<0>();
     }
-
-    const int ew = warp - 4;
-    const int q = ew & 3, half = ew >> 2;
-    const int col0 = tc.n_blk * BLOCK_N + half * (BLOCK_N / 2);
-    constexpr int NCH = BLOCK_N / 2 / 16;
-    constexpr int RPI = 32 / NCH;
-    constexpr bool kRowPerLane = EPI == EPI_DELTA;
-    auto wrow_of = [&](int j) { return kRowPerLane ? lane : RPI * j + lane % RPI; };
-    auto chunk_of = [&](int j) { return kRowPerLane ? j : lane / RPI; };
-    const long long gp_warp_off =
-        ((((static_cast<long long>(tc.m_blk >> 1) * n_blocks + tc.n_blk) * 2 + (tc.m_blk & 1)) * kEpiWarps + ew) * NCH) * 512;
-    auto gp_off = [&](int j) { return gp_warp_off + chunk_of(j) * 512 + wrow_of(j) * 16; };
-    constexpr bool kEx = !OUT_F32 && EPI != EPI_BIAS && !epi_is_gelu(EPI) && EPI != EPI_GELU_ONLY;
-    uint32_t ex[kEx ? NCH : 1][8];
-    if constexpr (kEx) {
-        constexpr bool kWantAdd = EPI == EPI_RESID || EPI == EPI_DROP_RESID || EPI == EPI_DELTA;
-        const int row0 = tc.m_blk * BLOCK_M + q * 32 + wrow_of(0), c0 = col0 + chunk_of(0) * 16;
-        const bf16* exb = nullptr;
-        long long ex_step = 0;
-        if (kWantAdd || (epi_is_generic(EPI) && p.addend != nullptr)) {
-            exb = p.addend + static_cast<long long>(row0) * p.ld_add + c0;
-            ex_step = kRowPerLane ? 16 : RPI * p.ld_add;
-        } else if (EPI == EPI_DGELU_BWD || (epi_is_generic(EPI) && p.epilogue == VB_EPI_DGELU)) {
-            exb = p.aux_in + static_cast<long long>(row0) * p.ld_aux + c0;
-            ex_step = kRowPerLane ? 16 : RPI * p.ld_aux;
-        } else if (EPI == EPI_DGELU_BWD_T) {
-            exb = p.aux_in + gp_off(0);
-            ex_step = kRowPerLane ? 512 : RPI * 16;
-        }
-#pragma unroll
-        for (int j = 0; j < NCH; ++j)
-            if (exb != nullptr && tc.m_blk * BLOCK_M + q * 32 + wrow_of(j) < p.M && col0 + chunk_of(j) * 16 < p.N) ldg_v8(exb + j * ex_step, ex[j]);
-    }
-
     named_bar_sync(1, kEpiWarps * 32);
-    float* sacc = reinterpret_cast<float*>(smem);
-    {
-        const int r0 = wg * 64 + ((warp & 3) << 4) + (lane >> 2);
-#pragma unroll
-        for (int h = 0; h < NH; ++h)
-#pragma unroll
-            for (int j = 0; j < 16; ++j)
+
+    if constexpr (OUT_F32) {
+        float* sacc = reinterpret_cast<float*>(smem);
+        {
+            const int r0 = wg * 64 + ((warp & 3) << 4) + (lane >> 2);
+#pragma unroll
+            for (int j = 0; j < BLOCK_N / 8; ++j)
 #pragma unroll
                 for (int i = 0; i < 2; ++i)
-                    *reinterpret_cast<float2*>(sacc + (r0 + 8 * i) * C::ACC_LD + h * 128 + j * 8 + 2 * (lane & 3)) =
-                        make_float2(acc[h][4 * j + 2 * i], acc[h][4 * j + 2 * i + 1]);
-    }
-    named_bar_sync(1, kEpiWarps * 32);
-
-    [[maybe_unused]] float hsum = 0.f;
-#pragma unroll
-    for (int k = 0; k < NCH; ++k) {
-        const int lrow = q * 32 + wrow_of(k), cc = half * (BLOCK_N / 2) + chunk_of(k) * 16;
-        const int row = tc.m_blk * BLOCK_M + lrow;
-        const int col = tc.n_blk * BLOCK_N + cc;
-        if (row < p.M && col < p.N) {
-            float x[16];
-#pragma unroll
-            for (int i = 0; i < 4; ++i) {
-                const float4 v = *reinterpret_cast<const float4*>(sacc + lrow * C::ACC_LD + cc + 4 * i);
-                x[4 * i] = v.x; x[4 * i + 1] = v.y; x[4 * i + 2] = v.z; x[4 * i + 3] = v.w;
-            }
-            const float* sb = has_bias ? sbias + cc : nullptr;
-            const uint32_t (&e)[8] = ex[kEx ? k : 0];
-            if constexpr (EPI == EPI_GELU_FWD_T) {
-                uint32_t o0[8], o1[8];
-                epilogue16<OUT_F32, EPI, true>(p, row, col, sb, e, x, o0, o1);
-                stg_v8(reinterpret_cast<bf16*>(p.D) + gp_off(k), o0);
-                stg_v8(p.aux_out + static_cast<long long>(row) * p.ld_aux + col, o1);
-            } else if constexpr (EPI == EPI_SLAB) {
-                float* d = reinterpret_cast<float*>(p.D) + (static_cast<long long>(blockIdx.x / (m_blocks * n_blocks)) * p.M + row) * p.ldd + col;
-#pragma unroll
-                for (int i = 0; i < 4; ++i) *reinterpret_cast<float4*>(d + 4 * i) = make_float4(x[4 * i], x[4 * i + 1], x[4 * i + 2], x[4 * i + 3]);
-            } else if constexpr (EPI == EPI_DELTA) {
-                uint32_t o0[8];
-                epilogue16<OUT_F32, EPI, true>(p, row, col, sb, e, x, o0);
-                stg_v8(reinterpret_cast<bf16*>(p.D) + static_cast<long long>(row) * p.ldd + col, o0);
-#pragma unroll
-                for (int i = 0; i < 8; ++i) {
-                    const float2 a = unpack_bf16x2(o0[i]), b = unpack_bf16x2(e[i]);
-                    hsum = fmaf(a.x, b.x, fmaf(a.y, b.y, hsum));
-                }
+                    *reinterpret_cast<float2*>(sacc + (r0 + 8 * i) * C::ACC_LD + j * 8 + 2 * (lane & 3)) =
+                        make_float2(acc[4 * j + 2 * i], acc[4 * j + 2 * i + 1]);
+        }
+        named_bar_sync(1, kEpiWarps * 32);
+        const int ew = warp - 4;
+        const int q = ew & 3, half = ew >> 2;
+        constexpr int NCH = BLOCK_N / 2 / 16;
+        constexpr int RPI = 32 / NCH;
+#pragma unroll
+        for (int k = 0; k < NCH; ++k) {
+            const int lrow = q * 32 + RPI * k + lane % RPI, cc = half * (BLOCK_N / 2) + (lane / RPI) * 16;
+            const int row = tc.m_blk * BLOCK_M + lrow;
+            const int col = tc.n_blk * BLOCK_N + cc;
+            if (row < p.M && col < p.N) {
+                float x[16];
+#pragma unroll
+                for (int i = 0; i < 4; ++i) {
+                    const float4 v = *reinterpret_cast<const float4*>(sacc + lrow * C::ACC_LD + cc + 4 * i);
+                    x[4 * i] = v.x; x[4 * i + 1] = v.y; x[4 * i + 2] = v.z; x[4 * i + 3] = v.w;
+                }
+                if constexpr (EPI == EPI_SLAB) {
+                    float* d = reinterpret_cast<float*>(p.D) + (static_cast<long long>(blockIdx.x / (m_blocks * n_blocks)) * p.M + row) * p.ldd + col;
+#pragma unroll
+                    for (int i = 0; i < 4; ++i) *reinterpret_cast<float4*>(d + 4 * i) = make_float4(x[4 * i], x[4 * i + 1], x[4 * i + 2], x[4 * i + 3]);
+                } else {
+                    if (has_bias) {
+#pragma unroll
+                        for (int i = 0; i < 4; ++i) {
+                            const float4 b = *reinterpret_cast<const float4*>(sbias + cc + 4 * i);
+                            x[4 * i] += b.x; x[4 * i + 1] += b.y; x[4 * i + 2] += b.z; x[4 * i + 3] += b.w;
+                        }
+                    }
+                    float* d = reinterpret_cast<float*>(p.D) + static_cast<long long>(row) * p.ldd + col;
+#pragma unroll
+                    for (int i = 0; i < 4; ++i) red_add_v4_f32(d + 4 * i, x[4 * i], x[4 * i + 1], x[4 * i + 2], x[4 * i + 3]);
+                }
+            }
+        }
+    } else {
+        constexpr bool kGeneric = epi_is_generic(EPI);
+        constexpr bool kTwoOut = epi_is_gelu(EPI) || kGeneric;
+        const bool two_out = epi_is_gelu(EPI) || (kGeneric && p.epilogue == VB_EPI_GELU);
+        const bool reads = epi_may_read(EPI) && epi_reads(EPI, p);
+        const bool is_dgelu = epi_is_dgelu(EPI) || (kGeneric && p.epilogue == VB_EPI_DGELU);
+        const bool add = EPI == EPI_RESID || EPI == EPI_DROP_RESID || (kGeneric && p.addend != nullptr);
+        const bool drop = EPI == EPI_DROP_RESID || (kGeneric && p.drop_scale != 0.0f);
+        const int w4 = warp & 3, qd = lane & 3;
+        const int frow0 = 64 * wg + 16 * w4 + (lane >> 2);
+        const int mrow = 64 * wg + 16 * w4 + ((lane >> 3) & 1) * 8 + (lane & 7);
+        const int mj = lane >> 4;
+        auto rm_addr = [&](int p0, int col) {
+            return piece_addr(p0 + (col >> 6)) + mrow * 128 + ((((col & 63) >> 3) ^ (mrow & 7)) << 4);
+        };
+        auto tn_addr = [&](int pbase, int col) {
+            const uint32_t o = tn_byte(mrow, col);
+            return piece_addr(pbase + (o >> 14)) + (o & (C::PIECE - 1));
+        };
+
+        constexpr int KW = BLOCK_N / 128;
+        uint32_t kw[2][KW];
+        if (drop) {
+            const uint32_t key0 = dropout_key(EPI == EPI_GENERIC_OFF ? p.drop_seed + *p.drop_offset : p.drop_seed, p.drop_stream);
+#pragma unroll
+            for (int i = 0; i < 2; ++i) {
+                const unsigned long long e0 =
+                    (static_cast<unsigned long long>(tc.m_blk * BLOCK_M + frow0 + 8 * i) * static_cast<unsigned>(p.N) + tc.n_blk * BLOCK_N) >> 3;
+#pragma unroll
+                for (int s = 0; s < KW; ++s) {
+                    uint32_t w = 0;
+#pragma unroll
+                    for (int b = 0; b < 4; ++b) w |= dropout_keep8_key(key0, e0 + 4 * (4 * s + b) + qd, p.drop_thresh16) << (8 * b);
+                    kw[i][s] = w;
+                }
+            }
+        }
+        uint32_t kq[2][KW][4];
+        if (drop) {
+#pragma unroll
+            for (int i = 0; i < 2; ++i)
+#pragma unroll
+                for (int s = 0; s < KW; ++s)
+#pragma unroll
+                    for (int q = 0; q < 4; ++q) kq[i][s][q] = __shfl_sync(0xffffffffu, kw[i][s], (lane & ~3) | q);
+        }
+        if (reads) mbar_wait(opnd_bar, 0);
+
+#pragma unroll
+        for (int jp = 0; jp < BLOCK_N / 16; ++jp) {
+            float* x = acc + 8 * jp;
+            const int mcol = 16 * jp + 8 * mj;
+            if (has_bias) {
+#pragma unroll
+                for (int k = 0; k < 4; ++k) {
+                    const float2 b = *reinterpret_cast<const float2*>(sbias + 8 * (2 * jp + k / 2) + 2 * qd);
+                    x[2 * k] += b.x; x[2 * k + 1] += b.y;
+                }
+            }
+            if (drop) {
+#pragma unroll
+                for (int k = 0; k < 4; ++k) {
+                    const int j = 2 * jp + k / 2;
+                    const uint32_t keep = kq[k % 2][j / 16][j & 3] >> (8 * ((j >> 2) & 3) + 2 * qd);
+                    x[2 * k] = (keep & 1u) ? x[2 * k] * p.drop_scale : 0.0f;
+                    x[2 * k + 1] = (keep & 2u) ? x[2 * k + 1] * p.drop_scale : 0.0f;
+                }
+            }
+            uint32_t e[4] = {0u, 0u, 0u, 0u};
+            if (reads) {
+                if (EPI == EPI_DGELU_BWD_T) ldmatrix_x4(tn_addr(0, mcol), e);
+                else ldmatrix_x4(rm_addr(0, mcol), e);
+            }
+            if (add) {
+#pragma unroll
+                for (int k = 0; k < 4; ++k) {
+                    const float2 t = unpack_bf16x2(e[k]);
+                    x[2 * k] += t.x;
+                    x[2 * k + 1] += t.y;
+                }
+            }
+            uint32_t o0[4], o1[4];
+            if (EPI == EPI_GELU_ONLY) {
+#pragma unroll
+                for (int k = 0; k < 8; ++k) {
+                    float gp;
+                    gelu_fwd_bwd(x[k], x[k], gp);
+                }
+            } else if (kTwoOut && two_out) {
+                float gp[8];
+#pragma unroll
+                for (int k = 0; k < 8; ++k) gelu_fwd_bwd(x[k], x[k], gp[k]);
+#pragma unroll
+                for (int k = 0; k < 4; ++k) o1[k] = pack_bf16x2(gp[2 * k], gp[2 * k + 1]);
+            } else if (is_dgelu) {
+#pragma unroll
+                for (int k = 0; k < 4; ++k) {
+                    const float2 t = unpack_bf16x2(e[k]);
+                    x[2 * k] *= t.x;
+                    x[2 * k + 1] *= t.y;
+                }
+            }
+#pragma unroll
+            for (int k = 0; k < 4; ++k) o0[k] = pack_bf16x2(x[2 * k], x[2 * k + 1]);
+            if (kTwoOut && two_out) {
+                stmatrix_x4(EPI == EPI_GELU_FWD_T ? tn_addr(C::OPND, mcol) : rm_addr(C::OPND, mcol), o1);
+                stmatrix_x4(rm_addr(2 * C::OPND, mcol), o0);
             } else {
-                epilogue16<OUT_F32, EPI>(p, row, col, sb, e, x);
+                stmatrix_x4(rm_addr(C::OPND, mcol), o0);
+            }
+            if ((jp & 3) == 3) {
+                fence_proxy_async_smem();
+                named_bar_sync(2 + wg, 128);
+                if ((threadIdx.x & 127) == 0) {
+                    const int b = jp >> 2, gcol = tc.n_blk * BLOCK_N + 64 * b, grow = tc.m_blk * BLOCK_M + 64 * wg;
+                    if (EPI == EPI_GELU_FWD_T) {
+                        if ((jp & 7) == 7) {
+                            const int pc = 2 * (jp >> 3) + wg;
+                            bulk_store(reinterpret_cast<uint8_t*>(p.D) + tn_tile * 2 + pc * C::PIECE, piece_addr(C::OPND + pc), C::PIECE);
+                        }
+                        tma_store_2d(&tmX, piece_addr(2 * C::OPND + b) + wg * 8192, gcol, grow);
+                    } else {
+                        tma_store_2d(&tmD, piece_addr(C::OPND + b) + wg * 8192, gcol, grow);
+                        if (kTwoOut && two_out) tma_store_2d(&tmX, piece_addr(2 * C::OPND + b) + wg * 8192, gcol, grow);
+                    }
+                    bulk_commit();
+                }
             }
         }
         if constexpr (EPI == EPI_DELTA) {
-            if ((k & 3) == 3) {
-                const int c4 = col - 48;
+            const int t = threadIdx.x & 127, r = 64 * wg + (t & 63), row = tc.m_blk * BLOCK_M + r;
+#pragma unroll
+            for (int hh = 0; hh < 2; ++hh) {
+                const int h = 2 * (t >> 6) + hh;
+                float sum = 0.f;
+#pragma unroll
+                for (int c = 0; c < 8; ++c) {
+                    const uint32_t off = r * 128 + ((c ^ (r & 7)) << 4);
+                    const uint4 dv = *reinterpret_cast<const uint4*>(smem + (piece_addr(C::OPND + h) - base) + off);
+                    const uint4 ov = *reinterpret_cast<const uint4*>(smem + (piece_addr(h) - base) + off);
+                    const uint32_t du[4] = {dv.x, dv.y, dv.z, dv.w}, ou[4] = {ov.x, ov.y, ov.z, ov.w};
+#pragma unroll
+                    for (int i = 0; i < 4; ++i) {
+                        const float2 x = unpack_bf16x2(du[i]), y = unpack_bf16x2(ou[i]);
+                        sum = fmaf(x.x, y.x, fmaf(x.y, y.y, sum));
+                    }
+                }
+                const int c4 = tc.n_blk * BLOCK_N + 64 * h;
                 if (row < p.M && c4 < p.N) {
                     const int bi = row / p.delta_seq, si = row - bi * p.delta_seq;
-                    p.delta_out[(static_cast<long long>(bi) * (p.N >> 6) + (c4 >> 6)) * p.delta_seq + si] = hsum;
-                }
-                hsum = 0.f;
-            }
-        }
+                    p.delta_out[(static_cast<long long>(bi) * (p.N >> 6) + (c4 >> 6)) * p.delta_seq + si] = sum;
+                }
+            }
+        }
+        if ((threadIdx.x & 127) == 0) bulk_wait_read0();
     }
 }
 
@@ -508,8 +577,10 @@
     return n[dev];
 }
 
+struct GemmMaps { CUtensorMap a, b, d, x, e; };
+
 template <bool A_MN, bool B_MN, int BLOCK_N, bool OUT_F32, int EPI = EPI_GENERIC>
-static int launch(const CUtensorMap& ta, const CUtensorMap& tb, const GemmParams& p, cudaStream_t st) {
+static int launch(const GemmMaps& m, const GemmParams& p, cudaStream_t st) {
     using C = Cfg<BLOCK_N>;
     auto kern = gemm_wgmma_kernel<A_MN, B_MN, BLOCK_N, OUT_F32, EPI>;
     static int configured[kMaxDevices] = {0};
@@ -518,7 +589,7 @@
     VB_REQUIRE(tiles < (1LL << 31), "vb_gemm: too many tiles");
     {
         ProfScope ps(st, OUT_F32 ? PROF_GEMM_WGRAD : (B_MN ? PROF_GEMM_DGRAD : PROF_GEMM_FWD), 2.0 * p.M * p.N * p.K, 1);
-        VB_CHECK_CUDA(launch_pdl(kern, dim3(static_cast<unsigned>(tiles)), dim3(kThreads), C::SMEM_BYTES, st, ta, tb, p));
+        VB_CHECK_CUDA(launch_pdl(kern, dim3(static_cast<unsigned>(tiles)), dim3(kThreads), C::SMEM_BYTES, st, m.a, m.b, p, m.d, m.x, m.e));
     }
     VB_CHECK_CUDA(cudaGetLastError());
     return 0;
@@ -592,9 +663,9 @@
                "vb_gemm: fp32-accumulate output supports bias only");
     VB_REQUIRE(a.dropout_p >= 0.0f && a.dropout_p < 1.0f, "vb_gemm: dropout_p out of range");
     VB_REQUIRE(!a.delta_out || (gemm_delta_ok(a.M, a.N) && a.delta_ctx && a.delta_seq > 0 && a.M % a.delta_seq == 0 && !a.d_fp32 &&
-                                !a.a_mn_major && a.b_mn_major && !a.bias && !a.addend && a.dropout_p == 0.0f && a.epilogue == VB_EPI_NONE &&
-                                (reinterpret_cast<uintptr_t>(a.delta_ctx) & 31) == 0),
+                                !a.a_mn_major && a.b_mn_major && !a.bias && !a.addend && a.dropout_p == 0.0f && a.epilogue == VB_EPI_NONE),
                "vb_gemm: delta_out needs a plain bf16 input-gradient GEMM (b_mn_major, no bias / addend / dropout) and vb_gemm_delta_ok(M, N)");
+    VB_REQUIRE(!a.delta_out || (reinterpret_cast<uintptr_t>(a.delta_ctx) & 31) == 0, "vb_gemm: delta_ctx must be 32-byte aligned");
     VB_REQUIRE(!a.gp_tiled || (gemm_gp_tiled_ok(a.M, a.N) && !a.d_fp32 && !a.a_mn_major && (a.epilogue == VB_EPI_GELU || a.epilogue == VB_EPI_DGELU)),
                "vb_gemm: gp_tiled needs a GELU / DGELU epilogue and vb_gemm_gp_tiled_ok(M, N)");
     VB_REQUIRE(!a.gp_tiled || a.epilogue != VB_EPI_DGELU || a.b_mn_major,
@@ -637,19 +708,23 @@
     }
     const bool slab = a.d_fp32 && p.splits > 1 && det.ptr != nullptr;
 
-    CUtensorMap ta, tb;
-    int rc;
-    if (!a.a_mn_major) rc = make_tmap_bf16(&ta, a.A, a.K, a.M, a.lda, BLOCK_M);
-    else               rc = make_tmap_bf16(&ta, a.A, a.M, a.K, a.lda, BLOCK_K);
-    if (rc) return rc;
-    if (!a.b_mn_major) rc = make_tmap_bf16(&tb, a.B, a.K, a.N, a.ldb, bn256 ? 256 : 128);
-    else               rc = make_tmap_bf16(&tb, a.B, a.N, a.K, a.ldb, BLOCK_K);
-    if (rc) return rc;
+    GemmMaps mp;
+    memset(&mp, 0, sizeof(mp));
+    if (!a.a_mn_major) VB_TRY_RC(make_tmap_bf16(&mp.a, a.A, a.K, a.M, a.lda, BLOCK_M));
+    else               VB_TRY_RC(make_tmap_bf16(&mp.a, a.A, a.M, a.K, a.lda, BLOCK_K));
+    if (!a.b_mn_major) VB_TRY_RC(make_tmap_bf16(&mp.b, a.B, a.K, a.N, a.ldb, bn256 ? 256 : 128));
+    else               VB_TRY_RC(make_tmap_bf16(&mp.b, a.B, a.N, a.K, a.ldb, BLOCK_K));
+    if (!a.d_fp32) {
+        if (!a.gp_tiled || a.epilogue != VB_EPI_GELU) VB_TRY_RC(make_tmap_bf16(&mp.d, a.D, a.N, a.M, a.ldd, 64));
+        if (a.aux_out) VB_TRY_RC(make_tmap_bf16(&mp.x, a.aux_out, a.N, a.M, a.ld_aux, 64));
+        if (p.addend) VB_TRY_RC(make_tmap_bf16(&mp.e, p.addend, a.N, a.M, p.ld_add, BLOCK_M));
+        else if (a.aux_in && !a.gp_tiled) VB_TRY_RC(make_tmap_bf16(&mp.e, a.aux_in, a.N, a.M, a.ld_aux, BLOCK_M));
+    }
 
     if (slab) {
         GemmParams q = p;
         q.D = det.ptr; q.ldd = a.N; q.bias = nullptr;
-        const int rc2 = bn256 ? launch<true, true, 256, true, EPI_SLAB>(ta, tb, q, st) : launch<true, true, 128, true, EPI_SLAB>(ta, tb, q, st);
+        const int rc2 = bn256 ? launch<true, true, 256, true, EPI_SLAB>(mp, q, st) : launch<true, true, 128, true, EPI_SLAB>(mp, q, st);
         if (rc2) return rc2;
         const long long n4 = static_cast<long long>(a.M) * a.N / 4;
         long long blocks = (n4 + 255) / 256;
@@ -664,7 +739,7 @@
     }
     if (off != nullptr) {
 #define VB_DISPATCH_OFF(AM, BM) \
-    (bn256 ? launch<AM, BM, 256, false, EPI_GENERIC_OFF>(ta, tb, p, st) : launch<AM, BM, 128, false, EPI_GENERIC_OFF>(ta, tb, p, st))
+    (bn256 ? launch<AM, BM, 256, false, EPI_GENERIC_OFF>(mp, p, st) : launch<AM, BM, 128, false, EPI_GENERIC_OFF>(mp, p, st))
         if (!a.a_mn_major && !a.b_mn_major) return VB_DISPATCH_OFF(false, false);
         if (!a.a_mn_major && a.b_mn_major) return VB_DISPATCH_OFF(false, true);
         if (a.a_mn_major && a.b_mn_major) return VB_DISPATCH_OFF(true, true);
@@ -672,7 +747,7 @@
 #undef VB_DISPATCH_OFF
     }
     if (a.epilogue == VB_EPI_GELU_FWD)
-        return bn256 ? launch<false, false, 256, false, EPI_GELU_ONLY>(ta, tb, p, st) : launch<false, false, 128, false, EPI_GELU_ONLY>(ta, tb, p, st);
+        return bn256 ? launch<false, false, 256, false, EPI_GELU_ONLY>(mp, p, st) : launch<false, false, 128, false, EPI_GELU_ONLY>(mp, p, st);
     if (bn256 && !a.d_fp32) {
         const bool drop = a.dropout_p > 0.0f, add = a.addend != nullptr;
         int epi = EPI_GENERIC;
@@ -682,28 +757,28 @@
         if (a.delta_out) epi = EPI_DELTA;
         if (!a.a_mn_major && !a.b_mn_major) {
             switch (epi) {
-                case EPI_BIAS: return launch<false, false, 256, false, EPI_BIAS>(ta, tb, p, st);
-                case EPI_RESID: return launch<false, false, 256, false, EPI_RESID>(ta, tb, p, st);
-                case EPI_DROP_RESID: return launch<false, false, 256, false, EPI_DROP_RESID>(ta, tb, p, st);
-                case EPI_GELU_FWD: return launch<false, false, 256, false, EPI_GELU_FWD>(ta, tb, p, st);
-                case EPI_GELU_FWD_T: return launch<false, false, 256, false, EPI_GELU_FWD_T>(ta, tb, p, st);
-                default: return launch<false, false, 256, false>(ta, tb, p, st);
+                case EPI_BIAS: return launch<false, false, 256, false, EPI_BIAS>(mp, p, st);
+                case EPI_RESID: return launch<false, false, 256, false, EPI_RESID>(mp, p, st);
+                case EPI_DROP_RESID: return launch<false, false, 256, false, EPI_DROP_RESID>(mp, p, st);
+                case EPI_GELU_FWD: return launch<false, false, 256, false, EPI_GELU_FWD>(mp, p, st);
+                case EPI_GELU_FWD_T: return launch<false, false, 256, false, EPI_GELU_FWD_T>(mp, p, st);
+                default: return launch<false, false, 256, false>(mp, p, st);
             }
         }
         if (!a.a_mn_major && a.b_mn_major) {
             switch (epi) {
-                case EPI_BIAS: return launch<false, true, 256, false, EPI_BIAS>(ta, tb, p, st);
-                case EPI_RESID: return launch<false, true, 256, false, EPI_RESID>(ta, tb, p, st);
-                case EPI_DGELU_BWD: return launch<false, true, 256, false, EPI_DGELU_BWD>(ta, tb, p, st);
-                case EPI_DELTA: return launch<false, true, 256, false, EPI_DELTA>(ta, tb, p, st);
-                case EPI_DGELU_BWD_T: return launch<false, true, 256, false, EPI_DGELU_BWD_T>(ta, tb, p, st);
-                default: return launch<false, true, 256, false>(ta, tb, p, st);
+                case EPI_BIAS: return launch<false, true, 256, false, EPI_BIAS>(mp, p, st);
+                case EPI_RESID: return launch<false, true, 256, false, EPI_RESID>(mp, p, st);
+                case EPI_DGELU_BWD: return launch<false, true, 256, false, EPI_DGELU_BWD>(mp, p, st);
+                case EPI_DELTA: return launch<false, true, 256, false, EPI_DELTA>(mp, p, st);
+                case EPI_DGELU_BWD_T: return launch<false, true, 256, false, EPI_DGELU_BWD_T>(mp, p, st);
+                default: return launch<false, true, 256, false>(mp, p, st);
             }
         }
     }
 
 #define VB_DISPATCH(AM, BM, F32)                                         \
-    (bn256 ? launch<AM, BM, 256, F32>(ta, tb, p, st) : launch<AM, BM, 128, F32>(ta, tb, p, st))
+    (bn256 ? launch<AM, BM, 256, F32>(mp, p, st) : launch<AM, BM, 128, F32>(mp, p, st))
     if (!a.d_fp32) {
         if (!a.a_mn_major && !a.b_mn_major) return VB_DISPATCH(false, false, false);
         if (!a.a_mn_major && a.b_mn_major) return VB_DISPATCH(false, true, false);
```

Measured after the change: 4566, median of 6. +5.8%, better.
